# ebanalyse/ebnerd-benchmark

Hardware: AMD Instinct MI355X
Metric: training impressions/sec (higher is better)
Workload: dtype f32

## Files before the change

### ebnerd-benchmark_amd/csrc/ebn_encoder.hip

```cpp
#include "ebn_common.h"

#define EBN_TRY(call)            \
  do {                           \
    int rc__ = (call);           \
    if (rc__ != EBN_OK) return rc__; \
  } while (0)

static int check_dims(const ebn_encoder_dims* d) {
  EBN_REQUIRE(d, EBN_ERR_BAD_ARG);
  EBN_REQUIRE(d->n_seq >= 0 && d->L > 0 && d->Din > 0 && d->h > 0 && d->d > 0 && d->A > 0, EBN_ERR_BAD_ARG);
  return EBN_OK;
}

extern "C" int ebn_encoder_fwd_f32(const ebn_encoder_dims* dims, const ebn_encoder_params* p,
                                   const ebn_encoder_acts* a, const ebn_encoder_scratch* s,
                                   const ebn_step_state* st, ebn_stream_t stream) {
  EBN_TRY(check_dims(dims));
  EBN_REQUIRE(p && a && p->Wqkv && p->W && p->b && p->q, EBN_ERR_BAD_ARG);
  EBN_REQUIRE(a->X && a->QKV && a->Y && a->U && a->w && a->out, EBN_ERR_BAD_ARG);
  const int64_t R = dims->n_seq * dims->L;
  const int E = dims->h * dims->d;
  if (R == 0) return EBN_OK;
  float* ws = s ? s->gemm_ws : nullptr;
  const int64_t ws_n = s ? s->gemm_ws_floats : 0;
  EBN_TRY(ebn_gemm_f32_site(0, 0, R, 3 * E, dims->Din, 1.0f, a->X, dims->Din, p->Wqkv, 3 * E, 0.0f, a->QKV, 3 * E, ws, ws_n,
                            1, stream));
  EBN_TRY(ebn_attn_fwd_f32(a->QKV, 3 * E, a->Y, E, dims->n_seq, dims->L, dims->h, dims->d, st, dims->drop_site,
                           dims->drop_p, stream));
  EBN_TRY(ebn_gemm_f32_ws(0, 0, R, dims->A, E, 1.0f, a->Y, E, p->W, dims->A, 0.0f, a->U, dims->A, ws, ws_n, stream));
  EBN_TRY(ebn_attpool_fwd_f32(a->U, p->b, p->q, a->Y, a->out, a->w, dims->n_seq, dims->L, E, dims->A, stream));
  return EBN_OK;
}

extern "C" int ebn_encoder_fwd_gather_f32(const ebn_encoder_dims* dims, const ebn_encoder_params* p, const ebn_encoder_acts* a,
                                          const ebn_encoder_scratch* s, const int32_t* ids, const float* table, int64_t table_rows,
                                          int32_t* oob_flag, ebn_stream_t stream) {
  EBN_TRY(check_dims(dims));
  EBN_REQUIRE(p && a && ids && table && p->Wqkv && p->W && p->b && p->q, EBN_ERR_BAD_ARG);
  EBN_REQUIRE(a->QKV && a->Y && a->U && a->w && a->out, EBN_ERR_BAD_ARG);
  EBN_REQUIRE(dims->drop_p <= 0.0f, EBN_ERR_UNSUPPORTED);
  const int64_t R = dims->n_seq * dims->L;
  const int E = dims->h * dims->d;
  if (R == 0) return EBN_OK;
  float* ws = s ? s->gemm_ws : nullptr;
  const int64_t ws_n = s ? s->gemm_ws_floats : 0;
  EBN_TRY(ebn_gemm_f32_rowmap(ids, table_rows, R, 3 * E, dims->Din, table, dims->Din, p->Wqkv, 3 * E, a->QKV, 3 * E, oob_flag, stream));
  EBN_TRY(ebn_attn_fwd_f32(a->QKV, 3 * E, a->Y, E, dims->n_seq, dims->L, dims->h, dims->d, nullptr, -1, 0.0f, stream));
  EBN_TRY(ebn_gemm_f32_ws(0, 0, R, dims->A, E, 1.0f, a->Y, E, p->W, dims->A, 0.0f, a->U, dims->A, ws, ws_n, stream));
  EBN_TRY(ebn_attpool_fwd_f32(a->U, p->b, p->q, a->Y, a->out, a->w, dims->n_seq, dims->L, E, dims->A, stream));
  return EBN_OK;
}

extern "C" int ebn_encoder_bwd_f32(const ebn_encoder_dims* dims, const ebn_encoder_params* p,
                                   const ebn_encoder_acts* a, const float* dout, const ebn_encoder_grads* g,
                                   const ebn_encoder_scratch* s, float* dX, int32_t accumulate,
                                   const ebn_step_state* st, ebn_stream_t stream) {
  EBN_TRY(check_dims(dims));
  EBN_REQUIRE(p && a && g && s && dout, EBN_ERR_BAD_ARG);
  EBN_REQUIRE(p->Wqkv && p->W && p->q, EBN_ERR_BAD_ARG);
  EBN_REQUIRE(a->X && a->QKV && a->Y && a->U && a->w, EBN_ERR_BAD_ARG);
  EBN_REQUIRE(g->dWqkv && g->dW && g->db && g->dq, EBN_ERR_BAD_ARG);
  EBN_REQUIRE(s->dY && s->dQKV && s->de && s->partials, EBN_ERR_BAD_ARG);
  const int64_t R = dims->n_seq * dims->L;
  const int E = dims->h * dims->d;
  const int A = dims->A;
  if (R == 0) return EBN_OK;
  const float beta = accumulate ? 1.0f : 0.0f;
  EBN_TRY(ebn_attpool_bwd_pool_f32(a->Y, a->w, dout, nullptr, s->de, dims->n_seq, dims->L, E, stream));
  EBN_TRY(ebn_attpool_bwd_dpre_f32(a->U, p->q, s->de, g->dq, g->db, s->partials, R, A, accumulate, stream));
  const bool fold = ebn_attn_bwd_pooled_supported(dims->L, dims->d) != 0 && (E % 4) == 0 && ebn_aligned16(dout) &&
                    ebn_aligned16(s->dY) && ebn_aligned16(a->QKV) && ebn_aligned16(s->dQKV);
  if (fold) {
    EBN_TRY(ebn_dense_bwd_pair_f32(R, E, A, a->Y, E, a->U, A, p->W, A, beta, g->dW, A, s->dY, E, s->gemm_ws, s->gemm_ws_floats,
                                   stream));
    EBN_TRY(ebn_attn_bwd_pooled_f32(a->QKV, 3 * E, s->dY, E, a->w, dout, E, s->dQKV, 3 * E, dims->n_seq, dims->L, dims->h,
                                    dims->d, st, dims->drop_site, dims->drop_p, stream));
  } else {
    EBN_TRY(ebn_gemm_f32_ws(1, 0, E, A, R, 1.0f, a->Y, E, a->U, A, beta, g->dW, A, s->gemm_ws, s->gemm_ws_floats, stream));
    EBN_TRY(ebn_gemm_f32_rank1(R, E, A, 1.0f, a->U, A, p->W, A, s->dY, E, a->w, dout, E, dims->L, s->gemm_ws,
                               s->gemm_ws_floats, stream));
    EBN_TRY(ebn_attn_bwd_f32(a->QKV, 3 * E, s->dY, E, s->dQKV, 3 * E, dims->n_seq, dims->L, dims->h, dims->d, st, dims->drop_site,
                             dims->drop_p, stream));
  }
  if (dX != nullptr)
    return ebn_dense_bwd_pair_f32(R, dims->Din, 3 * E, a->X, dims->Din, s->dQKV, 3 * E, p->Wqkv, 3 * E, beta, g->dWqkv, 3 * E, dX,
                                  dims->Din, s->gemm_ws, s->gemm_ws_floats, stream);
  EBN_TRY(ebn_gemm_f32_ws(1, 0, dims->Din, 3 * E, R, 1.0f, a->X, dims->Din, s->dQKV, 3 * E, beta, g->dWqkv, 3 * E,
                          s->gemm_ws, s->gemm_ws_floats, stream));
  return EBN_OK;
}

extern "C" int ebn_user_stage_train_f32(const ebn_encoder_dims* dims, const ebn_encoder_params* p, const ebn_encoder_acts* a,
                                        const float* cand, const float* labels, float* scores, float* probs, float* loss_rows,
                                        float* loss_out, float* dcand, float* duser, const ebn_encoder_grads* g,
                                        const ebn_encoder_scratch* s, float* head_partials, float* dX, int32_t C,
                                        int32_t loss_kind, float inv_batch, const ebn_step_state* st, ebn_stream_t stream) {
  EBN_TRY(check_dims(dims));
  EBN_REQUIRE(p && a && g && s && cand && labels && scores && probs && loss_rows && loss_out && dcand && duser && dX, EBN_ERR_BAD_ARG);
  EBN_REQUIRE(p->Wqkv && p->W && p->b && p->q && a->X && a->QKV && a->Y && a->U && a->w && a->out, EBN_ERR_BAD_ARG);
  EBN_REQUIRE(g->dWqkv && g->dW && g->db && g->dq && s->dY && s->dQKV && s->de && s->partials, EBN_ERR_BAD_ARG);
  EBN_REQUIRE(C > 0 && dims->drop_p <= 0.0f, EBN_ERR_BAD_ARG);
  const int64_t B = dims->n_seq, R = dims->n_seq * dims->L;
  const int E = dims->h * dims->d, A = dims->A, L = dims->L;
  if (R == 0) return EBN_OK;
  const bool fused = head_partials != nullptr && ebn_user_head_supported(L, C, E, A) != 0 &&
                     ebn_attn_bwd_pooled_supported(L, dims->d) != 0 && ebn_aligned16(a->U) && ebn_aligned16(a->Y) &&
                     ebn_aligned16(cand) && ebn_aligned16(dcand) && ebn_aligned16(duser) && ebn_aligned16(a->out) &&
                     ebn_aligned16(p->b) && ebn_aligned16(p->q) && ebn_aligned16(s->dY) && ebn_aligned16(a->QKV) &&
                     ebn_aligned16(s->dQKV);
  if (!fused) {
    EBN_TRY(ebn_encoder_fwd_f32(dims, p, a, s, st, stream));
    EBN_TRY(ebn_score_loss_train_f32(cand, a->out, labels, scores, probs, loss_rows, loss_out, dcand, duser, B, C, E, loss_kind,
                                     inv_batch, stream));
    return ebn_encoder_bwd_f32(dims, p, a, duser, g, s, dX, 0, st, stream);
  }
  float* ws = s->gemm_ws;
  const int64_t ws_n = s->gemm_ws_floats;
  EBN_TRY(ebn_gemm_f32_site(0, 0, R, 3 * E, dims->Din, 1.0f, a->X, dims->Din, p->Wqkv, 3 * E, 0.0f, a->QKV, 3 * E, ws, ws_n, 1, stream));
  EBN_TRY(ebn_attn_fwd_f32(a->QKV, 3 * E, a->Y, E, B, L, dims->h, dims->d, nullptr, -1, 0.0f, stream));
  EBN_TRY(ebn_gemm_f32_ws(0, 0, R, A, E, 1.0f, a->Y, E, p->W, A, 0.0f, a->U, A, ws, ws_n, stream));
  EBN_TRY(ebn_user_head_train_f32(a->U, p->b, p->q, a->Y, cand, labels, a->w, a->out, scores, probs, loss_rows, loss_out, dcand,
                                  duser, s->de, g->dq, g->db, head_partials, B, L, C, E, A, loss_kind, inv_batch, stream));
  EBN_TRY(ebn_dense_bwd_pair_f32(R, E, A, a->Y, E, a->U, A, p->W, A, 0.0f, g->dW, A, s->dY, E, ws, ws_n, stream));
  EBN_TRY(ebn_attn_bwd_pooled_f32(a->QKV, 3 * E, s->dY, E, a->w, duser, E, s->dQKV, 3 * E, B, L, dims->h, dims->d, nullptr, -1, 0.0f,
                                  stream));
  return ebn_dense_bwd_pair_f32(R, dims->Din, 3 * E, a->X, dims->Din, s->dQKV, 3 * E, p->Wqkv, 3 * E, 0.0f, g->dWqkv, 3 * E, dX,
                                dims->Din, ws, ws_n, stream);
}
```

### ebnerd-benchmark_amd/csrc/ebn_finish.hip

```cpp
#include "ebn_common.h"
#include "ebn_finish.h"
#include "ebn_reduce.h"

namespace {

struct FinishJobs {
  ebn_finish_job job[EBN_FINISH_MAX_JOBS];
  int32_t first_block[EBN_FINISH_MAX_JOBS + 1];
  int32_t n;
};

struct FinishAdam {
  EbnAdamFlat adam;
  int32_t n_rest;
  int64_t rest_off[EBN_ADAM_FLAT_MAX_REST];
  int64_t rest_len[EBN_ADAM_FLAT_MAX_REST];
  int64_t rest_total;
};
constexpr int REST_PER_BLOCK = 4096;

template <bool ADAM>
__device__ __forceinline__ void grad_finish_body(const FinishJobs& js, const FinishAdam* fa) {
  __shared__ float sm[32][33];
  const EbnAdamFlat* ad = ADAM ? &fa->adam : nullptr;
  if (ADAM && static_cast<int>(blockIdx.x) >= js.first_block[js.n]) {
    const float al = ad->st->adam_alpha;
    const int64_t e0 = static_cast<int64_t>(static_cast<int>(blockIdx.x) - js.first_block[js.n]) * REST_PER_BLOCK;
    for (int64_t e = e0 + threadIdx.x; e < e0 + REST_PER_BLOCK && e < fa->rest_total; e += 1024) {
      int64_t off = e;
      int r = 0;
      while (r + 1 < fa->n_rest && off >= fa->rest_len[r]) off -= fa->rest_len[r++];
      off += fa->rest_off[r];
      ebn_adam_flat_apply(*ad, al, off, ad->grad[off]);
    }
    return;
  }
  int j = 0;
  while (j + 1 < js.n && static_cast<int>(blockIdx.x) >= js.first_block[j + 1]) ++j;
  const ebn_finish_job& q = js.job[j];
  const int blk = static_cast<int>(blockIdx.x) - js.first_block[j], nblk = js.first_block[j + 1] - js.first_block[j];
  if (q.kind == EBN_FINISH_SPLITK) {
    ebn_splitk_sum_body(static_cast<uint32_t>(blk) * 1024u + threadIdx.x, static_cast<uint32_t>(nblk) * 1024u, q.partials, q.n_parts,
                        static_cast<uint32_t>(q.rows * q.cols), static_cast<uint32_t>(q.cols), q.beta, q.out0, q.ld, nullptr, nullptr, 0, 1, nullptr, ad);
  } else if (q.kind == EBN_FINISH_COLRED) {
    ebn_reduce_partials_body(sm, blk, q.partials, q.n_parts, 2, static_cast<int>(q.cols), q.scale, q.out0, q.out1, q.beta != 0.f ? 1 : 0, nullptr,
                             nullptr, ad);
  } else {
    ebn_user_head_finish_body(&sm[0][0], blk, nblk, q.partials, q.rows, static_cast<int>(q.cols), q.out0, q.out1, q.loss_rows, q.loss_out);
    if (ADAM && blk < nblk - 1 && threadIdx.x < 256) {
      const int idx = blk * 256 + static_cast<int>(threadIdx.x), A = static_cast<int>(q.cols);
      if (idx < 2 * A) {
        float* gp = (idx / A == 0 ? q.out0 : q.out1) + (idx % A);
        ebn_adam_flat_apply(*ad, ad->st->adam_alpha, gp - ad->grad, *gp);
      }
    }
  }
}

__global__ __launch_bounds__(1024) void grad_finish_kernel(FinishJobs js) { grad_finish_body<false>(js, nullptr); }
__global__ __launch_bounds__(1024) void grad_finish_adam_kernel(FinishJobs js, FinishAdam fa) { grad_finish_body<true>(js, &fa); }

}

static int plan_jobs(const ebn_finish_job* jobs, int32_t n_jobs, FinishJobs& js) {
  EBN_REQUIRE(n_jobs >= 0 && n_jobs <= EBN_FINISH_MAX_JOBS && (jobs != nullptr || n_jobs == 0), EBN_ERR_BAD_ARG);
  js.n = 0;
  js.first_block[0] = 0;
  for (int32_t i = 0; i < n_jobs; ++i) {
    const ebn_finish_job& q = jobs[i];
    EBN_REQUIRE(q.kind >= EBN_FINISH_SPLITK && q.kind <= EBN_FINISH_HEAD && q.rows >= 0 && q.cols >= 0 && q.n_parts >= 0, EBN_ERR_BAD_ARG);
    if (q.rows == 0 || q.cols == 0) continue;
    EBN_REQUIRE(q.partials && q.out0, EBN_ERR_BAD_ARG);
    int64_t blocks;
    if (q.kind == EBN_FINISH_SPLITK) {
      EBN_REQUIRE(q.n_parts >= 1 && q.ld >= q.cols, EBN_ERR_BAD_ARG);
      EBN_REQUIRE(q.rows * q.cols < (int64_t{1} << 31), EBN_ERR_UNSUPPORTED);
      blocks = ebn_ceil_div(q.rows * q.cols, 1024);
      if (blocks > 16384) blocks = 16384;
    } else if (q.kind == EBN_FINISH_COLRED) {
      EBN_REQUIRE(q.out1 && q.cols < (1 << 24), EBN_ERR_BAD_ARG);
      blocks = ebn_ceil_div(2 * q.cols, 32);
    } else {
      EBN_REQUIRE(q.out1 && q.loss_rows && q.loss_out && q.cols < (1 << 24), EBN_ERR_BAD_ARG);
      blocks = ebn_ceil_div(2 * q.cols, 256) + 1;
    }
    js.job[js.n] = q;
    js.first_block[js.n + 1] = js.first_block[js.n] + static_cast<int32_t>(blocks);
    ++js.n;
  }
  return EBN_OK;
}

extern "C" int ebn_grad_finish_f32(const ebn_finish_job* jobs, int32_t n_jobs, ebn_stream_t stream) {
  FinishJobs js;
  const int rc = plan_jobs(jobs, n_jobs, js);
  if (rc != EBN_OK) return rc;
  if (js.n == 0) return EBN_OK;
  EBN_LAUNCH(grad_finish_kernel, dim3(static_cast<unsigned>(js.first_block[js.n])), dim3(1024), 0, ebn_stream(stream), js);
  EBN_CHECK_LAUNCH();
  return EBN_OK;
}

extern "C" int ebn_grad_finish_adam_f32(const ebn_finish_job* jobs, int32_t n_jobs, const ebn_adam_flat* a, const ebn_step_state* st,
                                        ebn_stream_t stream) {
  EBN_REQUIRE(a != nullptr && st != nullptr && a->theta && a->grad && a->m && a->v && a->numel > 0, EBN_ERR_BAD_ARG);
  EBN_REQUIRE(a->n_rest >= 0 && a->n_rest <= EBN_ADAM_FLAT_MAX_REST, EBN_ERR_BAD_ARG);
  FinishJobs js;
  const int rc = plan_jobs(jobs, n_jobs, js);
  if (rc != EBN_OK) return rc;
  auto inside = [&](const float* p, int64_t count) { return p >= a->grad && count >= 0 && (p - a->grad) + count <= a->numel; };
  for (int i = 0; i < js.n; ++i) {
    const ebn_finish_job& q = js.job[i];
    if (q.kind == EBN_FINISH_SPLITK) EBN_REQUIRE(inside(q.out0, (q.rows - 1) * q.ld + q.cols), EBN_ERR_BAD_ARG);
    else EBN_REQUIRE(inside(q.out0, q.cols) && inside(q.out1, q.cols), EBN_ERR_BAD_ARG);
  }
  FinishAdam fa{};
  fa.adam = EbnAdamFlat{a->grad, a->theta, a->m, a->v, st, static_cast<float>(1.0 - a->beta1), static_cast<float>(1.0 - a->beta2),
                        static_cast<float>(a->eps), a->grad_scale};
  fa.n_rest = a->n_rest;
  for (int i = 0; i < a->n_rest; ++i) {
    EBN_REQUIRE(a->rest_off[i] >= 0 && a->rest_len[i] >= 0 && a->rest_off[i] + a->rest_len[i] <= a->numel, EBN_ERR_BAD_ARG);
    fa.rest_off[i] = a->rest_off[i];
    fa.rest_len[i] = a->rest_len[i];
    fa.rest_total += a->rest_len[i];
  }
  const int64_t blocks = js.first_block[js.n] + ebn_ceil_div(fa.rest_total, REST_PER_BLOCK);
  EBN_REQUIRE(blocks < (int64_t{1} << 30), EBN_ERR_UNSUPPORTED);
  if (blocks == 0) return EBN_OK;
  EBN_LAUNCH(grad_finish_adam_kernel, dim3(static_cast<unsigned>(blocks)), dim3(1024), 0, ebn_stream(stream), js, fa);
  EBN_CHECK_LAUNCH();
  return EBN_OK;
}
```

### ebnerd-benchmark_amd/csrc/ebn_userhead.hip

```cpp
#include "ebn_common.h"
#include "ebn_finish.h"

namespace {

constexpr int HEAD_THREADS = 1024;
constexpr float HEAD_KERAS_EPS = 1e-7f;

struct HeadArgs {
  float* U;
  const float* b;
  const float* q;
  const float* X;
  const float* cand;
  const float* labels;
  float* w;
  float* user;
  float* scores;
  float* probs;
  float* loss_rows;
  float* dcand;
  float* duser;
  float* de;
  float* partials;
  int L, C, E, A, loss_kind;
  float inv_batch;
};

__device__ __forceinline__ float head_bce_probs(float p, float y, float* dldp) {
  const float lo = HEAD_KERAS_EPS, hi = 1.0f - HEAD_KERAS_EPS;
  const bool in_range = p >= lo && p <= hi;
  const float pc = fminf(fmaxf(p, lo), hi);
  const float a = pc + HEAD_KERAS_EPS, bb = 1.0f - pc + HEAD_KERAS_EPS;
  *dldp = in_range ? (-(y / a) + (1.0f - y) / bb) : 0.f;
  return -(y * logf(a) + (1.0f - y) * logf(bb));
}

__global__ __launch_bounds__(HEAD_THREADS) void user_head_train_kernel(HeadArgs a) {
  extern __shared__ __attribute__((aligned(16))) float sm[];
  const int L = a.L, C = a.C, E = a.E, A = a.A;
  float* T = sm;
  float* Xs = T + L * A;
  float* Cs = Xs + L * E;
  float* us = Cs + C * E;
  float* du = us + E;
  float* ev = du + E;
  float* dwv = ev + L;
  float* sc = dwv + L;
  float* dsv = sc + C;
  const int64_t bi = blockIdx.x;
  const int tid = threadIdx.x, lane = tid & 63, wave = tid >> 6;
  const int A4 = A >> 2, E4 = E >> 2;
  {
    const float4* Ug = reinterpret_cast<const float4*>(a.U + bi * L * A);
    const float4* Xg = reinterpret_cast<const float4*>(a.X + bi * L * E);
    const float4* Cg = reinterpret_cast<const float4*>(a.cand + bi * C * E);
    const float4* bg = reinterpret_cast<const float4*>(a.b);
    constexpr int NB = 2;
    for (int base = 0; base < L * E4; base += HEAD_THREADS * NB) {
      float4 v[NB];
#pragma unroll
      for (int j = 0; j < NB; ++j) {
        const int i = base + j * HEAD_THREADS + tid;
        v[j] = Xg[i < L * E4 ? i : L * E4 - 1];
      }
#pragma unroll
      for (int j = 0; j < NB; ++j) {
        const int i = base + j * HEAD_THREADS + tid;
        if (i < L * E4) reinterpret_cast<float4*>(Xs)[i] = v[j];
      }
    }
    for (int base = 0; base < C * E4; base += HEAD_THREADS * NB) {
      float4 v[NB];
#pragma unroll
      for (int j = 0; j < NB; ++j) {
        const int i = base + j * HEAD_THREADS + tid;
        v[j] = Cg[i < C * E4 ? i : C * E4 - 1];
      }
#pragma unroll
      for (int j = 0; j < NB; ++j) {
        const int i = base + j * HEAD_THREADS + tid;
        if (i < C * E4) reinterpret_cast<float4*>(Cs)[i] = v[j];
      }
    }
    for (int base = 0; base < L * A4; base += HEAD_THREADS * NB) {
      float4 v[NB], bb[NB];
#pragma unroll
      for (int j = 0; j < NB; ++j) {
        const int i = base + j * HEAD_THREADS + tid;
        const int ic = i < L * A4 ? i : L * A4 - 1;
        v[j] = Ug[ic];
        bb[j] = bg[ic % A4];
      }
#pragma unroll
      for (int j = 0; j < NB; ++j) {
        const int i = base + j * HEAD_THREADS + tid;
        float4 t;
        t.x = tanhf(v[j].x + bb[j].x);
        t.y = tanhf(v[j].y + bb[j].y);
        t.z = tanhf(v[j].z + bb[j].z);
        t.w = tanhf(v[j].w + bb[j].w);
        if (i < L * A4) reinterpret_cast<float4*>(T)[i] = t;
      }
    }
  }
  __syncthreads();
  for (int l = wave; l < L; l += HEAD_THREADS / 64) {
    float part = 0.f;
    for (int k4 = lane; k4 < A4; k4 += 64) {
      const float4 t = reinterpret_cast<const float4*>(T + l * A)[k4];
      const float4 qq = reinterpret_cast<const float4*>(a.q)[k4];
      part = fmaf(t.w, qq.w, fmaf(t.z, qq.z, fmaf(t.y, qq.y, fmaf(t.x, qq.x, part))));
    }
    part = ebn_wave_sum(part);
    if (lane == 0) ev[l] = part;
  }
  __syncthreads();
  if (wave == 0) {
    float s = 0.f;
    for (int l = lane; l < L; l += 64) {
      const float ex = expf(ev[l]);
      ev[l] = ex;
      s += ex;
    }
    s = ebn_wave_sum(s) + HEAD_KERAS_EPS;
    for (int l = lane; l < L; l += 64) {
      const float wl = ev[l] / s;
      ev[l] = wl;
      a.w[bi * L + l] = wl;
    }
  }
  __syncthreads();
  for (int c4 = tid; c4 < E4; c4 += HEAD_THREADS) {
    float4 acc = make_float4(0.f, 0.f, 0.f, 0.f);
    for (int l = 0; l < L; ++l) {
      const float wl = ev[l];
      const float4 x = reinterpret_cast<const float4*>(Xs + l * E)[c4];
      acc.x = fmaf(wl, x.x, acc.x);
      acc.y = fmaf(wl, x.y, acc.y);
      acc.z = fmaf(wl, x.z, acc.z);
      acc.w = fmaf(wl, x.w, acc.w);
    }
    reinterpret_cast<float4*>(us)[c4] = acc;
    reinterpret_cast<float4*>(a.user + bi * E)[c4] = acc;
  }
  __syncthreads();
  for (int c = wave; c < C; c += HEAD_THREADS / 64) {
    float part = 0.f;
    for (int e4 = lane; e4 < E4; e4 += 64) {
      const float4 x = reinterpret_cast<const float4*>(Cs + c * E)[e4];
      const float4 u = reinterpret_cast<const float4*>(us)[e4];
      part = fmaf(x.w, u.w, fmaf(x.z, u.z, fmaf(x.y, u.y, fmaf(x.x, u.x, part))));
    }
    part = ebn_wave_sum(part);
    if (lane == 0) sc[c] = part;
  }
  __syncthreads();
  if (wave == 0) {
    const float* y = a.labels + bi * C;
    float mx = -INFINITY, ysum = 0.f;
    for (int c = lane; c < C; c += 64) {
      mx = fmaxf(mx, sc[c]);
      ysum += y[c];
    }
    mx = ebn_wave_max(mx);
    ysum = ebn_wave_sum(ysum);
    float se = 0.f;
    for (int c = lane; c < C; c += 64) se += expf(sc[c] - mx);
    se = ebn_wave_sum(se);
    const float lse = mx + logf(se);
    const float invbc = a.inv_batch / static_cast<float>(C);
    float loss = 0.f, dot = 0.f;
    for (int c = lane; c < C; c += 64) {
      const float s = sc[c];
      a.scores[bi * C + c] = s;
      const float p = expf(s - mx) / se;
      a.probs[bi * C + c] = p;
      float ds;
      if (a.loss_kind == 0) {
        const float logp = s - lse;
        loss -= y[c] * logp;
        ds = (expf(logp) * ysum - y[c]) * a.inv_batch;
      } else if (a.loss_kind == 1) {
        loss += fmaxf(s, 0.f) - s * y[c] + log1pf(expf(-fabsf(s)));
        ds = (1.0f / (1.0f + expf(-s)) - y[c]) * invbc;
      } else {
        loss += head_bce_probs(p, y[c], &ds);
        dot = fmaf(p, ds, dot);
      }
      dsv[c] = ds;
    }
    if (a.loss_kind == 2) {
      dot = ebn_wave_sum(dot);
      for (int c = lane; c < C; c += 64) dsv[c] = (expf(sc[c] - mx) / se) * (dsv[c] - dot) * invbc;
    }
    loss = ebn_wave_sum(loss) * (a.loss_kind == 0 ? a.inv_batch : invbc);
    if (lane == 0) a.loss_rows[bi] = loss;
  }
  __syncthreads();
  for (int e4 = tid; e4 < E4; e4 += HEAD_THREADS) {
    const float4 u = reinterpret_cast<const float4*>(us)[e4];
    float4 acc = make_float4(0.f, 0.f, 0.f, 0.f);
    for (int c = 0; c < C; ++c) {
      const float ds = dsv[c];
      const float4 x = reinterpret_cast<const float4*>(Cs + c * E)[e4];
      acc.x = fmaf(ds, x.x, acc.x);
      acc.y = fmaf(ds, x.y, acc.y);
      acc.z = fmaf(ds, x.z, acc.z);
      acc.w = fmaf(ds, x.w, acc.w);
      reinterpret_cast<float4*>(a.dcand + (bi * C + c) * E)[e4] = make_float4(ds * u.x, ds * u.y, ds * u.z, ds * u.w);
    }
    reinterpret_cast<float4*>(du)[e4] = acc;
    reinterpret_cast<float4*>(a.duser + bi * E)[e4] = acc;
  }
  __syncthreads();
  for (int l = wave; l < L; l += HEAD_THREADS / 64) {
    float part = 0.f;
    for (int e4 = lane; e4 < E4; e4 += 64) {
      const float4 x = reinterpret_cast<const float4*>(Xs + l * E)[e4];
      const float4 g = reinterpret_cast<const float4*>(du)[e4];
      part = fmaf(g.w, x.w, fmaf(g.z, x.z, fmaf(g.y, x.y, fmaf(g.x, x.x, part))));
    }
    part = ebn_wave_sum(part);
    if (lane == 0) dwv[l] = part;
  }
  __syncthreads();
  if (wave == 0) {
    float s = 0.f;
    for (int l = lane; l < L; l += 64) s = fmaf(ev[l], dwv[l], s);
    s = ebn_wave_sum(s);
    for (int l = lane; l < L; l += 64) {
      const float d = ev[l] * (dwv[l] - s);
      dwv[l] = d;
      a.de[bi * L + l] = d;
    }
  }
  __syncthreads();
  for (int k = tid; k < A; k += HEAD_THREADS) {
    const float qk = a.q[k];
    float dq = 0.f, db = 0.f;
    for (int l = 0; l < L; ++l) {
      const float t = T[l * A + k], d = dwv[l];
      dq = fmaf(d, t, dq);
      const float dp = d * qk * (1.0f - t * t);
      a.U[(bi * L + l) * A + k] = dp;
      db += dp;
    }
    a.partials[(bi * 2 + 0) * A + k] = dq;
    a.partials[(bi * 2 + 1) * A + k] = db;
  }
}

__global__ __launch_bounds__(256) void user_head_finish_kernel(const float* __restrict__ partials, int64_t B, int A,
                                                               float* __restrict__ dq, float* __restrict__ db,
                                                               const float* __restrict__ loss_rows,
                                                               float* __restrict__ loss_out) {
  __shared__ float sw[4];
  ebn_user_head_finish_body(sw, blockIdx.x, gridDim.x, partials, B, A, dq, db, loss_rows, loss_out);
}

size_t head_lds_bytes(int L, int C, int E, int A) {
  return sizeof(float) * (static_cast<size_t>(L) * A + static_cast<size_t>(L) * E + static_cast<size_t>(C) * E + 2 * static_cast<size_t>(E) +
                          2 * static_cast<size_t>(L) + 2 * static_cast<size_t>(C));
}

}

extern "C" int ebn_user_head_supported(int32_t L, int32_t C, int32_t E, int32_t A) {
  if (L <= 0 || C <= 0 || E <= 0 || A <= 0 || (E % 4) != 0 || (A % 4) != 0) return 0;
  return head_lds_bytes(L, C, E, A) <= 150 * 1024 ? 1 : 0;
}

extern "C" int64_t ebn_user_head_partials_len(int64_t B, int32_t A) { return ebn_dim_ok(B, A) ? B * 2 * static_cast<int64_t>(A) : 0; }

extern "C" int ebn_user_head_train_f32(float* U, const float* b, const float* q, const float* X, const float* cand,
                                       const float* labels, float* w, float* user, float* scores, float* probs,
                                       float* loss_rows, float* loss_out, float* dcand, float* duser, float* de, float* dq,
                                       float* db, float* partials, int64_t B, int32_t L, int32_t C, int32_t E, int32_t A,
                                       int32_t loss_kind, float inv_batch, ebn_stream_t stream) {
  EBN_REQUIRE(U && b && q && X && cand && labels && w && user && scores && probs && loss_rows && loss_out && dcand && duser &&
                  de && partials && ((dq != nullptr) == (db != nullptr)),
              EBN_ERR_BAD_ARG);
  EBN_REQUIRE(B >= 0 && L > 0 && C > 0 && E > 0 && A > 0, EBN_ERR_BAD_ARG);
  EBN_REQUIRE(loss_kind >= 0 && loss_kind <= 2 && ebn_user_head_supported(L, C, E, A), EBN_ERR_UNSUPPORTED);
  EBN_REQUIRE(ebn_aligned16(U) && ebn_aligned16(b) && ebn_aligned16(q) && ebn_aligned16(X) && ebn_aligned16(cand) &&
                  ebn_aligned16(user) && ebn_aligned16(dcand) && ebn_aligned16(duser),
              EBN_ERR_ALIGN);
  if (B == 0) return EBN_OK;
  hipStream_t s = ebn_stream(stream);
  const size_t lds = head_lds_bytes(L, C, E, A);
  static const hipError_t attr = hipFuncSetAttribute(reinterpret_cast<const void*>(&user_head_train_kernel),
                                                     hipFuncAttributeMaxDynamicSharedMemorySize, 150 * 1024);
  if (attr != hipSuccess) return static_cast<int>(attr);
  HeadArgs a{U, b, q, X, cand, labels, w, user, scores, probs, loss_rows, dcand, duser, de, partials, L, C, E, A, loss_kind, inv_batch};
  EBN_LAUNCH(user_head_train_kernel, dim3(static_cast<unsigned>(B)), dim3(HEAD_THREADS), lds, s, a);
  EBN_CHECK_LAUNCH();
  if (dq == nullptr) return EBN_OK;
  EBN_LAUNCH(user_head_finish_kernel, dim3(static_cast<unsigned>(ebn_ceil_div(2 * A, 256) + 1)), dim3(256), 0, s, partials, B, A,
                     dq, db, loss_rows, loss_out);
  EBN_CHECK_LAUNCH();
  return EBN_OK;
}
```

### ebnerd-benchmark_amd/ebrec/models/newsrec/_engine.py

```python
from __future__ import annotations

import ctypes
import math

import numpy as np
import torch

from ebrec import _hip

BETA1, BETA2, ADAM_EPS = 0.9, 0.999, 1e-7
_ALIGN = 64

from ._engine_segments import SegmentsMixin
from ._engine_staging import StagingMixin

LOSS_KIND = {"cross_entropy_loss": 0, "log_loss": 1}
BCE_ON = ("logits", "probs")


def loss_kind_of(loss: str, bce_on: str) -> int:
    if bce_on not in BCE_ON:
        raise ValueError(f"bce_on must be one of {BCE_ON}, got {bce_on}")
    return 0 if loss == "cross_entropy_loss" else (1 if bce_on == "logits" else 2)


def require_gpu() -> torch.device:
    if not torch.cuda.is_available():
        raise RuntimeError("the MI355X NRMS path needs a visible GPU (no CPU fallback); "
                           "torch.cuda.is_available() is False")
    _hip.lib()
    return torch.device("cuda", torch.cuda.current_device())


def eval_loss_from_news(eng, news_all: torch.Tensor, his_idx, pred_idx, y):
    his_idx, pred_idx = np.asarray(his_idx), np.asarray(pred_idx)
    B, C = his_idx.shape[0], pred_idx.shape[1]
    H, E = his_idx.shape[1], eng.E
    idx = torch.from_numpy(np.ascontiguousarray(np.concatenate([his_idx.reshape(-1), pred_idx.reshape(-1)]), dtype=np.int32)).to(eng.device)
    NE = torch.empty(B * (H + C), E, device=eng.device)
    S = _hip.stream_handle
    _hip.call("ebn_gather_rows_f32", _hip.ptr(idx), _hip.ptr(news_all), _hip.ptr(NE), B * (H + C), E, news_all.shape[0], None, -1,
              ctypes.c_float(0.0), None, S())
    user = eng.encode_users_from_news(NE[: B * H].view(B, H, E))
    cand = NE[B * H:]
    scores, probs = torch.empty(B, C, device=eng.device), torch.empty(B, C, device=eng.device)
    _hip.call("ebn_score_fwd_f32", _hip.ptr(cand), _hip.ptr(user), _hip.ptr(scores), _hip.ptr(probs), B, C, E, 0, S())
    labels = (y if isinstance(y, torch.Tensor) else torch.from_numpy(np.ascontiguousarray(np.asarray(y, dtype=np.float32))))
    labels = labels.to(device=eng.device, dtype=torch.float32).reshape(B, C).contiguous()
    rows, junk_c, junk_u = torch.empty(B, device=eng.device), torch.empty(B * C, E, device=eng.device), torch.empty(B, E, device=eng.device)
    loss = torch.empty(1, device=eng.device)
    _hip.call("ebn_score_loss_bwd_f32", _hip.ptr(cand), _hip.ptr(user), _hip.ptr(scores), _hip.ptr(labels), _hip.ptr(rows),
              _hip.ptr(junk_c), _hip.ptr(junk_u), B, C, E, eng.loss_kind, ctypes.c_float(1.0 / B), S())
    _hip.call("ebn_sum_f32", _hip.ptr(rows), B, ctypes.c_float(1.0), _hip.ptr(loss), 0, S())
    return loss, probs


def glorot_uniform_np(shape, seed):
    rng = np.random.default_rng(seed)
    lim = math.sqrt(6.0 / (shape[0] + shape[-1]))
    return rng.uniform(-lim, lim, size=shape).astype(np.float32)


class FlatParams:

    def __init__(self, shapes: dict, device):
        self.shapes = dict(shapes)
        self.offsets = {}
        off = 0
        for name, shp in shapes.items():
            self.offsets[name] = off
            off += -(-int(np.prod(shp)) // _ALIGN) * _ALIGN
        self.numel = off
        self.data = torch.zeros(off, device=device)
        self.grad = torch.zeros(off, device=device)
        self.m = torch.zeros(off, device=device)
        self.v = torch.zeros(off, device=device)

    def view(self, name, buf=None):
        buf = self.data if buf is None else buf
        n = int(np.prod(self.shapes[name]))
        return buf[self.offsets[name]: self.offsets[name] + n].view(*self.shapes[name])

    def g(self, name):
        return self.view(name, self.grad)


class EncoderBuffers:

    def __init__(self, n_seq, L, Din, E, A, device, own_input, need_dx):
        R = n_seq * L
        self.n_seq, self.L, self.Din, self.E, self.A, self.R = n_seq, L, Din, E, A, R
        f = lambda *s: torch.empty(*s, device=device)
        self.X = f(R, Din) if own_input else None
        self.QKV, self.Y, self.U, self.w = f(R, 3 * E), f(R, E), f(R, A), f(R)
        self.out = f(n_seq, E)
        self.dY, self.dQKV, self.de = f(R, E), f(R, 3 * E), f(R)
        self.partials = f(int(_hip.lib().ebn_attpool_partials_len(R, A)))
        wsf = _hip.lib().ebn_gemm_workspace_floats
        ws = max(int(wsf(Din, 3 * E, R)), int(wsf(E, A, R)), int(wsf(R, 3 * E, Din)), int(wsf(R, A, E)), int(wsf(R, E, A)),
                 int(wsf(R, Din, 3 * E)), 1)
        self.ws = f(ws)
        self.fwd_scratch = _hip.EncoderScratch(None, None, None, None, self.ws.data_ptr(), self.ws.numel())
        self.dX = f(R, Din) if need_dx else None


class NRMSEngine(StagingMixin, SegmentsMixin):
    def __init__(self, table: np.ndarray, title_size: int, history_size: int, head_num: int, head_dim: int,
                 attention_hidden_dim: int, dropout: float, learning_rate: float, loss: str, seed=None,
                 train_embedding: bool = True, device=None, process_group=None, shard_table: bool = False,
                 shard_mode: str = "alltoall", deterministic: bool = True, units=None, l2: float = 0.0,
                 shard_partition: str | None = None, shard_capacity_factor: float = 1.25, table_grad_exchange: str = "auto",
                 bce_on: str = "logits", precision: str = "exact"):
        self.device = require_gpu() if device is None else torch.device(device)
        if precision not in ("exact", "split"):
            raise ValueError(f"precision must be 'exact' (fp32 MFMA, the default) or 'split' (bf16x6 split on the bf16 matrix pipe, "
                             f"fp32-accurate, fp32 accumulate), got {precision}")
        self.precision = precision
        if loss not in LOSS_KIND:
            raise ValueError(f"this loss not defined {loss}")
        loss_kind_of(loss, bce_on)
        self.bce_on = bce_on
        self.T, self.H = int(title_size), int(history_size)
        self.h, self.d, self.A = int(head_num), int(head_dim), int(attention_hidden_dim)
        self.E = self.h * self.d
        self.p = float(dropout)
        self.loss = loss
        self.seed = seed
        self.train_embedding = bool(train_embedding)
        if table_grad_exchange not in ("auto", "dense", "sparse"):
            raise ValueError(f"table_grad_exchange must be auto | dense | sparse, got {table_grad_exchange}")
        self.table_grad_exchange = table_grad_exchange
        self._sparse_pin = None
        self.pg = process_group
        table = np.ascontiguousarray(table, dtype=np.float32)
        self.V, self.D = table.shape
        self.exchange = None
        if shard_table:
            from ._dist import ShardedTableExchange

            self.exchange = ShardedTableExchange(self.V, self.D, group=process_group, mode=shard_mode, partition=shard_partition,
                                                 capacity_factor=shard_capacity_factor)
            table = self.exchange.shard_of(table)
        self.table = torch.from_numpy(np.ascontiguousarray(table)).to(self.device)
        D, E, A = self.D, self.E, self.A
        self.units = [int(u) for u in units] if units else []
        if self.units and self.precision == "split":
            raise ValueError("precision='split' covers the news encoder without the optional per-token Dense stack "
                             "(newsencoder_units_per_layer); use precision='exact' with it")
        if self.units and self.units[-1] != E:
            raise ValueError(f"newsencoder_units_per_layer must end with head_num*head_dim = {E} (the news vector is dotted with "
                             f"the {E}-wide user vector, nrms.py:201), got {self.units}")
        shapes = {"n_Wqkv": (D, 3 * E)}
        if self.units:
            from ._mlp import MLPStack

            shapes.update(MLPStack.shapes("n_", E, self.units))
        shapes.update({"n_W": (E, A), "n_b": (A,), "n_q": (A,), "u_Wqkv": (E, 3 * E), "u_W": (E, A), "u_b": (A,), "u_q": (A,)})
        self.params = FlatParams(shapes, self.device)
        self._graphs = {}
        self.mlp = MLPStack(self.params, "n_", E, self.units, self.device, l2, on_realloc=lambda: self._graphs.clear()) if self.units else None
        self._init_weights(seed)
        self.deterministic = bool(deterministic)
        if self.train_embedding:
            self.table_grad = torch.zeros_like(self.table)
            self.table_m = torch.zeros_like(self.table)
            self.table_v = torch.zeros_like(self.table)
            if self.deterministic:
                self.table_acc = torch.zeros(self.table.shape, dtype=torch.int64, device=self.device)
        st = _hip.StepState()
        st.step, st.seed, st.lr, st.adam_alpha = 0, (0 if seed is None else int(seed)) & 0xFFFFFFFF, learning_rate, 0.0
        self.state = torch.frombuffer(bytearray(bytes(st)), dtype=torch.uint8).to(self.device)
        self._lr = float(learning_rate)
        self._bufs = {}
        self.oob_flag = torch.zeros(1, dtype=torch.int32, device=self.device)
        self.keep_table_grad = False
        self.range_flag = torch.zeros(1, dtype=torch.int32, device=self.device)
        self.loss_dev = torch.zeros(1, device=self.device)
        self.use_graph = False
        self.fuse_user_head = True
        self.fuse_eval_gather = True
        self.defer_finish = True
        self.atomic_table_grad = False
        self.graph_collectives = False
        self.overlap_collectives = True
        self.skip_collectives = False
        self._pending = []
        self.defer_flag_checks = False
        self.trace = None
        self.world = 1
        if process_group is not None or (torch.distributed.is_available() and torch.distributed.is_initialized()):
            self.world = torch.distributed.get_world_size(process_group)
        self.guard = None
        if self.world > 1:
            from ._dist import LockStepGuard

            self.guard = LockStepGuard(process_group)
        self.force_collectives = False
        self.adam_in_finish = True
        self._adam_done_in_finish = False

    @property
    def multi(self) -> bool:
        return self.world > 1 or self.force_collectives

    @property
    def loss_kind(self) -> int:
        return loss_kind_of(self.loss, self.bce_on)

    def _init_weights(self, seed):
        D, E, A = self.D, self.E, self.A
        s = (lambda: seed) if seed is not None else (lambda: None)
        pv = self.params.view
        with torch.no_grad():
            for pre, din in (("n", D), ("u", E)):
                w = np.concatenate([glorot_uniform_np((din, E), s()) for _ in range(3)], axis=1)
                pv(f"{pre}_Wqkv").copy_(torch.from_numpy(w))
                pv(f"{pre}_W").copy_(torch.from_numpy(glorot_uniform_np((E, A), s())))
                pv(f"{pre}_b").zero_()
                pv(f"{pre}_q").copy_(torch.from_numpy(glorot_uniform_np((A, 1), s())[:, 0]))
        if self.mlp is not None:
            self.mlp.init_weights((lambda k: None) if seed is None else (lambda k: int(seed) * 1000 + k), glorot_uniform_np)

    def weight_names(self):
        base = ["news.emb", "news.attn.WQ", "news.attn.WK", "news.attn.WV"]
        if self.mlp is not None:
            base += self.mlp.weight_names("news")
        return base + ["news.att.W", "news.att.b", "news.att.q", "user.attn.WQ", "user.attn.WK", "user.attn.WV", "user.att.W",
                       "user.att.b", "user.att.q"]

    def get_weights(self):
        E = self.E
        out = [self._full_table().cpu().numpy()]
        for pre in ("n", "u"):
            w = self.params.view(f"{pre}_Wqkv").cpu().numpy()
            out += [w[:, :E].copy(), w[:, E:2 * E].copy(), w[:, 2 * E:].copy()]
            if pre == "n" and self.mlp is not None:
                out += self.mlp.get_weights()
            out += [self.params.view(f"{pre}_W").cpu().numpy(), self.params.view(f"{pre}_b").cpu().numpy(),
                    self.params.view(f"{pre}_q").cpu().numpy().reshape(-1, 1)]
        return out

    def set_weights(self, weights):
        n_mlp = 6 * len(self.units)
        if len(weights) != 13 + n_mlp:
            raise ValueError(f"expected {13 + n_mlp} weight arrays (emb, 2x[WQ,WK,WV,W,b,q]{' + 6 per Dense/BN layer' if n_mlp else ''}), "
                             f"got {len(weights)}")
        w = [np.asarray(a, dtype=np.float32) for a in weights]
        if n_mlp:
            self.mlp.set_weights([torch.from_numpy(np.ascontiguousarray(a)) for a in w[4:4 + n_mlp]])
            w = w[:4] + w[4 + n_mlp:]
        if w[0].shape != (self.V, self.D):
            raise ValueError(f"embedding shape {w[0].shape} != {(self.V, self.D)}")
        with torch.no_grad():
            t0 = w[0] if self.exchange is None else self.exchange.shard_of(w[0])
            self.table.copy_(torch.from_numpy(np.ascontiguousarray(t0)))
            i = 1
            for pre in ("n", "u"):
                self.params.view(f"{pre}_Wqkv").copy_(torch.from_numpy(np.concatenate(w[i:i + 3], axis=1)))
                self.params.view(f"{pre}_W").copy_(torch.from_numpy(w[i + 3]))
                self.params.view(f"{pre}_b").copy_(torch.from_numpy(w[i + 4].reshape(-1)))
                self.params.view(f"{pre}_q").copy_(torch.from_numpy(w[i + 5].reshape(-1)))
                i += 6

    def _full_table(self) -> torch.Tensor:
        if self.exchange is None or self.exchange.world == 1:
            return self.table
        per = self.exchange.per
        mine = torch.zeros(per, self.D, device=self.device)
        mine[: self.table.shape[0]] = self.table
        parts = [torch.empty_like(mine) for _ in range(self.exchange.world)]
        torch.distributed.all_gather(parts, mine, group=self.pg)
        return self.exchange.unshard(parts)

    def count_params(self):
        return self.V * self.D + sum(int(np.prod(s)) for s in self.params.shapes.values()) + 2 * sum(self.units)

    @property
    def _planned(self) -> bool:
        return self.exchange is not None and self.exchange.mode == "alltoall"

    @property
    def _adam_from_acc(self) -> bool:
        return (self.train_embedding and self.deterministic and self.exchange is None and not self.multi
                and not self.keep_table_grad)

    def _sparse_dp(self, n_tok: int) -> bool:
        if not (self.multi and self.train_embedding and self.exchange is None and self.deterministic and not self.keep_table_grad):
            return False
        if self.table_grad_exchange != "auto":
            return self.table_grad_exchange == "sparse"
        return self.pin_table_grad_exchange(n_tok)

    def pin_table_grad_exchange(self, n_tok_full: int) -> bool:
        if self._sparse_pin is None:
            self._sparse_pin = bool(self.world * int(n_tok_full) < self.V)
        return self._sparse_pin

    @property
    def needs_equal_batches(self) -> bool:
        if self.world <= 1:
            return False
        if self.exchange is not None:
            return True
        if not (self.train_embedding and self.deterministic and not self.keep_table_grad):
            return False
        if self.table_grad_exchange != "auto":
            return self.table_grad_exchange == "sparse"
        return True if self._sparse_pin is None else self._sparse_pin

    @property
    def graph_capable(self) -> bool:
        return self.exchange is None or self._planned

    def allreduce_bytes(self, n_tok: int = 0) -> int:
        n = self.params.numel * 4
        if self.train_embedding and self.exchange is None:
            n += n_tok * (4 + self.D * 4) if self._sparse_dp(n_tok) else self.table_grad.numel() * 4
        return n

    def enable_graphs(self, flag=True):
        self.use_graph = bool(flag)
        if not flag:
            self._graphs = {}
        return self

    @property
    def learning_rate(self):
        return self._lr

    @learning_rate.setter
    def learning_rate(self, lr):
        self._lr = float(lr)
        st = self.read_state()
        st.lr = self._lr
        self.state.copy_(torch.frombuffer(bytearray(bytes(st)), dtype=torch.uint8))

    def read_state(self):
        return _hip.StepState.from_buffer_copy(self.state.cpu().numpy().tobytes())

    def _news_bufs(self, N, train):
        key = ("news", train)
        b = self._bufs.get(key)
        if b is None or b.n_seq < N:
            b = EncoderBuffers(N, self.T, self.D, self.E, self.A, self.device, own_input=True,
                               need_dx=train and self.train_embedding)
            b.ids = torch.empty(N * self.T, dtype=torch.int32, device=self.device)
            if self._planned:
                from ._dist import PlannedBuffers

                ws = int(_hip.lib().ebn_shard_plan_workspace_ints(self.V, self.exchange.world))
                b.xb = PlannedBuffers(self.exchange, N * self.T, self.device, need_grad=train and self.train_embedding, ws_ints=ws)
            self._bufs[key] = b
            if train:
                self._graphs.clear()
        return b

    def _user_bufs(self, B, train, H=None):
        H = self.H if H is None else int(H)
        key = ("user", train) if H == self.H else ("user", train, H)
        b = self._bufs.get(key)
        if b is None or b.n_seq < B:
            b = EncoderBuffers(B, H, self.E, self.E, self.A, self.device, own_input=False, need_dx=False)
            self._bufs[key] = b
            if train and H == self.H:
                self._graphs.clear()
        return b

    def _enc_structs(self, pre, b: EncoderBuffers, n_seq, X, drop_site, drop_p):
        pv = self.params.view
        dims = _hip.EncoderDims(n_seq, b.L, b.Din, self.h, self.d, self.A, drop_site, drop_p)
        params = _hip.EncoderParams(pv(f"{pre}_Wqkv").data_ptr(), pv(f"{pre}_W").data_ptr(),
                                    pv(f"{pre}_b").data_ptr(), pv(f"{pre}_q").data_ptr())
        acts = _hip.EncoderActs(X.data_ptr(), b.QKV.data_ptr(), b.Y.data_ptr(), b.U.data_ptr(), b.w.data_ptr(),
                                b.out.data_ptr())
        return dims, params, acts

    def _encoder_fwd(self, pre, b, n_seq, X, train, n_first=None):
        site, p = (1, self.p) if (train and pre == "n" and self.p > 0) else (-1, 0.0)
        st = _hip.ptr(self.state) if train else None
        if pre == "n" and self.mlp is not None:
            return self._news_encoder_fwd_mlp(b, n_seq, X, train, n_seq if n_first is None else n_first)
        if pre == "n" and self.precision == "split":
            return self._news_encoder_fwd_split(b, n_seq, X, st, site, p)
        dims, params, acts = self._enc_structs(pre, b, n_seq, X, site, p)
        _hip.call("ebn_encoder_fwd_f32", ctypes.byref(dims), ctypes.byref(params), ctypes.byref(acts),
                  ctypes.byref(self._fwd_scratch(b)), st, _hip.stream_handle())

    @staticmethod
    def _fwd_scratch(b):
        return b.fwd_scratch

    def _news_encoder_fwd_mlp(self, b, n_seq, X, train, n_first):
        S, E, A, T = _hip.stream_handle, self.E, self.A, b.L
        R = n_seq * T
        pv = self.params.view
        _hip.call("ebn_gemm_f32_site", 0, 0, R, 3 * E, b.Din, ctypes.c_float(1.0), _hip.ptr(X), b.Din, _hip.ptr(pv("n_Wqkv")), 3 * E,
                  ctypes.c_float(0.0), _hip.ptr(b.QKV), 3 * E, _hip.ptr(b.ws), b.ws.numel(), 1, S())
        _hip.call("ebn_attn_fwd_f32", _hip.ptr(b.QKV), 3 * E, _hip.ptr(b.Y), E, n_seq, T, self.h, self.d, None, -1, ctypes.c_float(0.0), S())
        b.Z = self.mlp.forward(b.Y, n_first * T, (n_seq - n_first) * T, train, self.state, self.p)
        _hip.call("ebn_gemm_f32_ws", 0, 0, R, A, E, ctypes.c_float(1.0), _hip.ptr(b.Z), E, _hip.ptr(pv("n_W")), A, ctypes.c_float(0.0),
                  _hip.ptr(b.U), A, _hip.ptr(b.ws), b.ws.numel(), S())
        _hip.call("ebn_attpool_fwd_f32", _hip.ptr(b.U), _hip.ptr(pv("n_b")), _hip.ptr(pv("n_q")), _hip.ptr(b.Z), _hip.ptr(b.out),
                  _hip.ptr(b.w), n_seq, T, E, A, S())

    def _news_encoder_bwd_mlp(self, b, n_seq, X, dout, dX, n_first):
        S, E, A, T = _hip.stream_handle, self.E, self.A, b.L
        R = n_seq * T
        pv, g = self.params.view, self.params.g
        ws, wsn = _hip.ptr(b.ws), b.ws.numel()
        one, zero = ctypes.c_float(1.0), ctypes.c_float(0.0)
        _hip.call("ebn_attpool_bwd_pool_f32", _hip.ptr(b.Z), _hip.ptr(b.w), _hip.ptr(dout), _hip.ptr(b.dY), _hip.ptr(b.de), n_seq, T, E, S())
        _hip.call("ebn_attpool_bwd_dpre_f32", _hip.ptr(b.U), _hip.ptr(pv("n_q")), _hip.ptr(b.de), _hip.ptr(g("n_q")), _hip.ptr(g("n_b")),
                  _hip.ptr(b.partials), R, A, 0, S())
        _hip.call("ebn_gemm_f32_ws", 1, 0, E, A, R, one, _hip.ptr(b.Z), E, _hip.ptr(b.U), A, zero, _hip.ptr(g("n_W")), A, ws, wsn, S())
        _hip.call("ebn_gemm_f32_ws", 0, 1, R, E, A, one, _hip.ptr(b.U), A, _hip.ptr(pv("n_W")), A, one, _hip.ptr(b.dY), E, ws, wsn, S())
        dYattn = self.mlp.backward(b.dY, b.Y, n_first * T, (n_seq - n_first) * T, self.state, self.p, need_dx0=True,
                                   loss_dev=self.loss_dev)
        _hip.call("ebn_attn_bwd_f32", _hip.ptr(b.QKV), 3 * E, _hip.ptr(dYattn), E, _hip.ptr(b.dQKV), 3 * E, n_seq, T, self.h, self.d,
                  None, -1, ctypes.c_float(0.0), S())
        _hip.call("ebn_gemm_f32_ws", 1, 0, b.Din, 3 * E, R, one, _hip.ptr(X), b.Din, _hip.ptr(b.dQKV), 3 * E, zero, _hip.ptr(g("n_Wqkv")),
                  3 * E, ws, wsn, S())
        if dX is not None:
            _hip.call("ebn_gemm_f32_ws", 0, 1, R, b.Din, 3 * E, one, _hip.ptr(b.dQKV), 3 * E, _hip.ptr(pv("n_Wqkv")), 3 * E, zero,
                      _hip.ptr(dX), b.Din, ws, wsn, S())

    def _split_ws(self, b):
        if getattr(b, "split_ws", None) is None:
            f = _hip.lib().ebn_gemm_prec_workspace_bytes
            R, E3, D = b.R, 3 * b.E, b.Din
            nbytes = max(int(f(R, E3, D, 1)), int(f(D, E3, R, 1)), int(f(R, D, E3, 1)) if b.dX is not None else 0)
            b.split_ws = torch.empty(nbytes // 4 + 64, device=self.device)
            b.split_ws_bytes = nbytes
        return b.split_ws

    def _split_bufs(self, b):
        sb = getattr(b, "split_bufs", None)
        if sb is None:
            L = _hip.lib()
            R, E3, D = b.R, 3 * b.E, b.Din
            u8 = lambda n: torch.empty(int(n) + 64, dtype=torch.uint8, device=self.device)
            sb = b.split_bufs = {"XN": u8(L.ebn_planes_bytes(R, D)), "XT": u8(L.ebn_planes_bytes(D, R)), "Wp": u8(L.ebn_planes_bytes(E3, D)),
                                 "dQp": u8(L.ebn_planes_bytes(E3, R)),
                                 "part": torch.empty(max(int(L.ebn_gemm_planes_workspace_floats(D, E3, R)), int(L.ebn_gemm_planes_workspace_floats(R, E3, D)), 1),
                                                     device=self.device)}
        return sb

    def _gemm_prec(self, b, tA, tB, M, N, K, A, lda, Bm, ldb, C, ldc):
        ws = self._split_ws(b)
        _hip.call("ebn_gemm_f32_prec", tA, tB, M, N, K, ctypes.c_float(1.0), _hip.ptr(A), lda, _hip.ptr(Bm), ldb, ctypes.c_float(0.0),
                  _hip.ptr(C), ldc, _hip.ptr(ws), b.split_ws_bytes, 1, _hip.stream_handle())

    def _news_encoder_fwd_split_gemm(self, b, R):
        S, E = _hip.stream_handle, self.E
        sb = self._split_bufs(b)
        _hip.call("ebn_split_planes_f32", _hip.ptr(self.params.view("n_Wqkv")), 3 * E, 3 * E, b.Din, 1, _hip.ptr(sb["Wp"]), S())
        _hip.call("ebn_gemm_planes_f32", _hip.ptr(sb["XN"]), R, _hip.ptr(sb["Wp"]), 3 * E, b.Din, ctypes.c_float(1.0), ctypes.c_float(0.0),
                  _hip.ptr(b.QKV), 3 * E, _hip.ptr(sb["part"]), sb["part"].numel(), S())

    def _news_encoder_fwd_split(self, b, n_seq, X, st, site, p):
        S, E, A, T = _hip.stream_handle, self.E, self.A, b.L
        R = n_seq * T
        pv = self.params.view
        if getattr(b, "planes_rows", -1) == R:
            self._news_encoder_fwd_split_gemm(b, R)
        else:
            self._gemm_prec(b, 0, 0, R, 3 * E, b.Din, X, b.Din, pv("n_Wqkv"), 3 * E, b.QKV, 3 * E)
        _hip.call("ebn_attn_fwd_f32", _hip.ptr(b.QKV), 3 * E, _hip.ptr(b.Y), E, n_seq, T, self.h, self.d, st, site, ctypes.c_float(p), S())
        _hip.call("ebn_gemm_f32_ws", 0, 0, R, A, E, ctypes.c_float(1.0), _hip.ptr(b.Y), E, _hip.ptr(pv("n_W")), A, ctypes.c_float(0.0),
                  _hip.ptr(b.U), A, _hip.ptr(b.ws), b.ws.numel(), S())
        _hip.call("ebn_attpool_fwd_f32", _hip.ptr(b.U), _hip.ptr(pv("n_b")), _hip.ptr(pv("n_q")), _hip.ptr(b.Y), _hip.ptr(b.out),
                  _hip.ptr(b.w), n_seq, T, E, A, S())

    def _news_encoder_bwd_split(self, b, n_seq, X, dout, dX, site, p):
        self._news_bwd_p1(b, n_seq, dout)
        self._news_bwd_p2(b, n_seq, X, dout, site, p)
        if dX is not None:
            self._news_bwd_p3(b, n_seq, dX)

    def _news_bwd_p1(self, b, n_seq, dout):
        S, E, A, T = _hip.stream_handle, self.E, self.A, b.L
        R = n_seq * T
        pv, g = self.params.view, self.params.g
        ws, wsn = _hip.ptr(b.ws), b.ws.numel()
        one, zero = ctypes.c_float(1.0), ctypes.c_float(0.0)
        _hip.call("ebn_attpool_bwd_pool_f32", _hip.ptr(b.Y), _hip.ptr(b.w), _hip.ptr(dout), None, _hip.ptr(b.de), n_seq, T, E, S())
        _hip.call("ebn_attpool_bwd_dpre_f32", _hip.ptr(b.U), _hip.ptr(pv("n_q")), _hip.ptr(b.de), _hip.ptr(g("n_q")), _hip.ptr(g("n_b")),
                  _hip.ptr(b.partials), R, A, 0, S())
        if self._fold_pooling(T):
            _hip.call("ebn_dense_bwd_pair_f32", R, E, A, _hip.ptr(b.Y), E, _hip.ptr(b.U), A, _hip.ptr(pv("n_W")), A, zero, _hip.ptr(g("n_W")), A,
                      _hip.ptr(b.dY), E, ws, wsn, S())
        else:
            _hip.call("ebn_gemm_f32_ws", 1, 0, E, A, R, one, _hip.ptr(b.Y), E, _hip.ptr(b.U), A, zero, _hip.ptr(g("n_W")), A, ws, wsn, S())
            _hip.call("ebn_gemm_f32_rank1", R, E, A, one, _hip.ptr(b.U), A, _hip.ptr(pv("n_W")), A, _hip.ptr(b.dY), E, _hip.ptr(b.w), _hip.ptr(dout), E,
                      T, ws, wsn, S())

    def _fold_pooling(self, T) -> bool:
        return int(_hip.lib().ebn_attn_bwd_pooled_supported(T, self.d)) != 0 and self.E % 4 == 0

    def _news_bwd_p2(self, b, n_seq, X, dout, site, p):
        S, E, T = _hip.stream_handle, self.E, b.L
        R = n_seq * T
        g = self.params.g
        st = _hip.ptr(self.state)
        one, zero = ctypes.c_float(1.0), ctypes.c_float(0.0)
        if self._fold_pooling(T):
            _hip.call("ebn_attn_bwd_pooled_f32", _hip.ptr(b.QKV), 3 * E, _hip.ptr(b.dY), E, _hip.ptr(b.w), _hip.ptr(dout), E, _hip.ptr(b.dQKV), 3 * E,
                      n_seq, T, self.h, self.d, st, site, ctypes.c_float(p), S())
        else:
            _hip.call("ebn_attn_bwd_f32", _hip.ptr(b.QKV), 3 * E, _hip.ptr(b.dY), E, _hip.ptr(b.dQKV), 3 * E, n_seq, T, self.h, self.d, st, site,
                      ctypes.c_float(p), S())
        if self.precision != "split":
            _hip.call("ebn_gemm_f32_ws", 1, 0, b.Din, 3 * E, R, one, _hip.ptr(X), b.Din, _hip.ptr(b.dQKV), 3 * E, zero, _hip.ptr(g("n_Wqkv")), 3 * E,
                      _hip.ptr(b.ws), b.ws.numel(), S())
        elif getattr(b, "planes_rows", -1) == R:
            sb = self._split_bufs(b)
            _hip.call("ebn_split_planes_f32", _hip.ptr(b.dQKV), 3 * E, 3 * E, R, 1, _hip.ptr(sb["dQp"]), S())
            _hip.call("ebn_gemm_planes_f32", _hip.ptr(sb["XT"]), b.Din, _hip.ptr(sb["dQp"]), 3 * E, R, one, zero, _hip.ptr(g("n_Wqkv")), 3 * E,
                      _hip.ptr(sb["part"]), sb["part"].numel(), S())
        else:
            self._gemm_prec(b, 1, 0, b.Din, 3 * E, R, X, b.Din, b.dQKV, 3 * E, g("n_Wqkv"), 3 * E)

    def _news_bwd_p3(self, b, n_seq, dX):
        E, R = self.E, n_seq * b.L
        pv = self.params.view
        if self.precision != "split":
            _hip.call("ebn_gemm_f32_ws", 0, 1, R, b.Din, 3 * E, ctypes.c_float(1.0), _hip.ptr(b.dQKV), 3 * E, _hip.ptr(pv("n_Wqkv")), 3 * E,
                      ctypes.c_float(0.0), _hip.ptr(dX), b.Din, _hip.ptr(b.ws), b.ws.numel(), _hip.stream_handle())
        else:
            self._gemm_prec(b, 0, 1, R, b.Din, 3 * E, b.dQKV, 3 * E, pv("n_Wqkv"), 3 * E, dX, b.Din)

    def roofline_kernels(self, B, C):
        N = B * (self.H + C)
        nb, _ub = self._train_bufs(B, C)
        S, E, R = _hip.stream_handle, self.E, N * self.T
        pv = self.params.view
        site, p = (0, self.p) if self.p > 0 else (-1, 0.0)
        st = _hip.ptr(self.state)

        def qkv_gemm():
            if self.precision == "split":
                nb.planes_rows = R
                return self._news_encoder_fwd_split_gemm(nb, R)
            _hip.call("ebn_gemm_f32_site", 0, 0, R, 3 * E, nb.Din, ctypes.c_float(1.0), _hip.ptr(nb.X), nb.Din,
                      _hip.ptr(pv("n_Wqkv")), 3 * E, ctypes.c_float(0.0), _hip.ptr(nb.QKV), 3 * E, _hip.ptr(nb.ws), nb.ws.numel(), 1, S())

        def make_gather(ids):
            table_rows = self.table.shape[0]
            src = ids if table_rows == self.V else torch.remainder(ids, table_rows).to(torch.int32)

            def gather():
                self._gather_tokens(nb, src, self.table, table_rows, R, st, site, p, True)

            return gather

        return {"qkv_gemm": qkv_gemm, "gather": make_gather}

    def _encoder_bwd(self, pre, b, n_seq, X, dout, dX, n_first=None):
        if pre == "n" and self.mlp is not None:
            return self._news_encoder_bwd_mlp(b, n_seq, X, dout, dX, n_seq if n_first is None else n_first)
        site, p = (1, self.p) if (pre == "n" and self.p > 0) else (-1, 0.0)
        if pre == "n" and self.precision == "split":
            return self._news_encoder_bwd_split(b, n_seq, X, dout, dX, site, p)
        dims, params, acts = self._enc_structs(pre, b, n_seq, X, site, p)
        g = self.params.g
        grads = _hip.EncoderGrads(g(f"{pre}_Wqkv").data_ptr(), g(f"{pre}_W").data_ptr(), g(f"{pre}_b").data_ptr(),
                                  g(f"{pre}_q").data_ptr())
        scratch = _hip.EncoderScratch(b.dY.data_ptr(), b.dQKV.data_ptr(), b.de.data_ptr(), b.partials.data_ptr(),
                                      b.ws.data_ptr(), b.ws.numel())
        _hip.call("ebn_encoder_bwd_f32", ctypes.byref(dims), ctypes.byref(params), ctypes.byref(acts), _hip.ptr(dout),
                  ctypes.byref(grads), ctypes.byref(scratch), _hip.ptr(dX), 0, _hip.ptr(self.state),
                  _hip.stream_handle())

    def _news_forward(self, b, N, train, n_first=None, looked_up=False):
        site, p = (0, self.p) if (train and self.p > 0) else (-1, 0.0)
        st = _hip.ptr(self.state) if train else None
        n_tok = N * self.T
        if self._planned:
            if not looked_up:
                for _kind, fn in self._lookup_segments(b, N):
                    fn()
            xb = b.xb
            self._gather_tokens(b, xb.inv, xb.rows, self.exchange.world * self.exchange.capacity(n_tok), n_tok, st, site, p, train)
            return self._encoder_fwd("n", b, N, b.X, train, n_first)
        if self.exchange is not None:
            b.plan = self.exchange.plan(b.ids[: n_tok])
            b.rows_uniq = self.exchange.lookup(b.plan, self._local_gather)
            self._gather_tokens(b, b.plan.inv, b.rows_uniq, b.rows_uniq.shape[0], n_tok, st, site, p, train)
            return self._encoder_fwd("n", b, N, b.X, train, n_first)
        if not train and self.fuse_eval_gather and self.mlp is None and self.precision == "exact":
            dims, params, acts = self._enc_structs("n", b, N, b.X, -1, 0.0)
            rc = _hip.lib().ebn_encoder_fwd_gather_f32(ctypes.byref(dims), ctypes.byref(params), ctypes.byref(acts), ctypes.byref(self._fwd_scratch(b)),
                                                       _hip.ptr(b.ids), _hip.ptr(self.table), self.V, _hip.ptr(self.oob_flag), _hip.stream_handle())
            if rc == 0:
                return
            if rc != -2:
                raise _hip.HipError(f"ebn_encoder_fwd_gather_f32 failed with code {rc}")
        self._gather_tokens(b, b.ids, self.table, self.V, n_tok, st, site, p, train)
        self._encoder_fwd("n", b, N, b.X, train, n_first)

    def _gather_tokens(self, b, ids, table, table_rows, n_tok, st, site, p, train):
        if self.precision == "split" and train and self.mlp is None and n_tok <= b.R:
            sb = self._split_bufs(b)
            _hip.call("ebn_gather_split_planes_f32", _hip.ptr(ids), _hip.ptr(table), n_tok, self.D, table_rows, st, site, ctypes.c_float(p),
                      _hip.ptr(self.oob_flag), _hip.ptr(sb["XN"]), _hip.ptr(sb["XT"]), _hip.stream_handle())
            b.planes_rows = n_tok
            return
        b.planes_rows = -1
        _hip.call("ebn_gather_rows_f32", _hip.ptr(ids), _hip.ptr(table), _hip.ptr(b.X), n_tok, self.D, table_rows, st, site,
                  ctypes.c_float(p), _hip.ptr(self.oob_flag), _hip.stream_handle())

    def encode_news(self, ids, chunk=8192) -> torch.Tensor:
        ids = ids if isinstance(ids, torch.Tensor) else np.asarray(ids)
        N = ids.shape[0]
        if ids.ndim != 2 or ids.shape[1] != self.T:
            raise ValueError(f"expected ids of shape (N, {self.T}), got {tuple(ids.shape)}")
        out = torch.empty(N, self.E, device=self.device)
        for s in range(0, N, chunk):
            n = min(chunk, N - s)
            b = self._news_bufs(min(chunk, N), False)
            self._upload_ids(b.ids, ids[s:s + n])
            self._news_forward(b, n, False)
            out[s:s + n].copy_(b.out[:n])
        self._check_oob()
        return out

    def encode_users_from_news(self, NEh: torch.Tensor) -> torch.Tensor:
        B, H = NEh.shape[0], NEh.shape[1]
        X = NEh.reshape(B * H, self.E).contiguous()
        b = self._user_bufs(B, False, H)
        self._encoder_fwd("u", b, B, X, False)
        return b.out[:B].clone()

    def encode_users(self, his) -> torch.Tensor:
        his = his if isinstance(his, torch.Tensor) else np.asarray(his)
        B, H = his.shape[0], his.shape[1]
        NEh = self.encode_news(his.reshape(B * H, self.T))
        return self.encode_users_from_news(NEh.view(B, H, self.E))

    def forward(self, his, pred, mode="softmax"):
        his = his if isinstance(his, torch.Tensor) else np.asarray(his)
        pred = pred if isinstance(pred, torch.Tensor) else np.asarray(pred)
        B, C = his.shape[0], pred.shape[1]
        self._check_shapes(his, pred)
        N = B * (self.H + C)
        nb = self._news_bufs(N, False)
        self._upload_ids(nb.ids, his, pred)
        self._news_forward(nb, N, False, B * self.H)
        ub = self._user_bufs(B, False)
        self._encoder_fwd("u", ub, B, nb.out, False)
        scores = torch.empty(B, C, device=self.device)
        probs = torch.empty(B, C, device=self.device)
        cand = nb.out[B * self.H:]
        _hip.call("ebn_score_fwd_f32", _hip.ptr(cand), _hip.ptr(ub.out), _hip.ptr(scores), _hip.ptr(probs), B, C,
                  self.E, 0 if mode == "softmax" else 1, _hip.stream_handle())
        self._check_oob()
        return probs, scores

    def eval_loss(self, his, pred, y):
        probs, scores = self.forward(his, pred, mode="softmax")
        B, C = scores.shape
        labels = (y if isinstance(y, torch.Tensor) else torch.from_numpy(np.ascontiguousarray(np.asarray(y, dtype=np.float32))))
        labels = labels.to(device=self.device, dtype=torch.float32).reshape(B, C).contiguous()
        nb, ub = self._news_bufs(B * (self.H + C), False), self._user_bufs(B, False)
        rows = torch.empty(B, device=self.device)
        junk_c = torch.empty(B * C, self.E, device=self.device)
        junk_u = torch.empty(B, self.E, device=self.device)
        loss = torch.empty(1, device=self.device)
        _hip.call("ebn_score_loss_bwd_f32", _hip.ptr(nb.out[B * self.H:]), _hip.ptr(ub.out), _hip.ptr(scores),
                  _hip.ptr(labels), _hip.ptr(rows), _hip.ptr(junk_c), _hip.ptr(junk_u), B, C, self.E,
                  self.loss_kind, ctypes.c_float(1.0 / B), _hip.stream_handle())
        _hip.call("ebn_sum_f32", _hip.ptr(rows), B, ctypes.c_float(1.0), _hip.ptr(loss), 0, _hip.stream_handle())
        return loss, probs

    def pair_scores(self, user, news, u_idx, n_idx, sigmoid=True):
        n = u_idx.numel()
        out = torch.empty(n, device=self.device)
        _hip.call("ebn_pair_score_f32", _hip.ptr(user), _hip.ptr(news), _hip.ptr(u_idx), _hip.ptr(n_idx),
                  _hip.ptr(out), n, self.E, 1 if sigmoid else 0, _hip.stream_handle())
        return out

    def _check_shapes(self, his, pred):
        if his.ndim != 3 or his.shape[1] != self.H or his.shape[2] != self.T:
            raise ValueError(f"his_input_title must be (B, {self.H}, {self.T}), got {tuple(his.shape)}")
        if pred.ndim != 3 or pred.shape[0] != his.shape[0] or pred.shape[2] != self.T:
            raise ValueError(f"pred_input_title must be (B, C, {self.T}), got {tuple(pred.shape)}")

    def _check_oob(self, collective=None):
        if collective is None:
            if self.defer_flag_checks:
                return
            collective = self.exchange is not None
        collective = bool(collective) and self.multi
        err = None
        if self._planned:
            for key in sorted((k for k, b in self._bufs.items() if hasattr(b, "xb")), key=repr):
                try:
                    self.exchange.check(self._bufs[key].xb, collective=collective)
                except Exception as e:
                    err = err or e
        flags = torch.cat([self.oob_flag, self.range_flag])
        if collective:
            torch.distributed.all_reduce(flags, op=torch.distributed.ReduceOp.MAX, group=self.pg)
        oob, rng_bad = (int(v) for v in flags.cpu().tolist())
        if oob or rng_bad or err is not None:
            self.oob_flag.zero_()
            self.range_flag.zero_()
        if err is not None:
            raise err
        if oob != 0:
            raise IndexError(f"token id out of range [0, {self.V}) for the embedding table")
        if rng_bad != 0:
            raise FloatingPointError("embedding gradient left the range of the deterministic fixed-point accumulator (|sum| >= 2^22 "
                                     "or NaN): the run has diverged; deterministic=False accumulates in fp32 instead")

    def check_oob(self):
        self._check_oob(collective=True)

    def sync_moving_statistics(self) -> None:
        if self.world > 1 and self.mlp is not None:
            self.mlp.sync_moving_statistics(self.pg)

    def l2_penalty(self) -> float:
        return self.mlp.l2_penalty() if self.mlp is not None else 0.0

    def train_step(self, his, pred, y, return_probs=False, indexed=False):
        his = his if isinstance(his, torch.Tensor) else np.asarray(his)
        pred = pred if isinstance(pred, torch.Tensor) else np.asarray(pred)
        B, C = his.shape[0], pred.shape[1]
        advanced = False
        if indexed:
            if his.ndim != 2 or his.shape[1] != self.H or pred.ndim != 2 or pred.shape[0] != B:
                raise ValueError(f"indexed batches must be (B, {self.H}) and (B, C), got {tuple(his.shape)} {tuple(pred.shape)}")
            nb, ub = self._train_bufs(B, C)
            y, advanced = self._stage_indexed(nb, his, pred, y)
        else:
            self._check_shapes(his, pred)
            nb, ub = self._train_bufs(B, C)
            if self._device_batch(his, pred, y):
                nh = his.numel()
                _hip.call("ebn_copy3_advance", _hip.ptr(his), _hip.ptr(nb.ids), nh * 4, _hip.ptr(pred), _hip.ptr(nb.ids[nh:]),
                          pred.numel() * 4, _hip.ptr(y), _hip.ptr(nb.labels), y.numel() * 4, _hip.ptr(self.state), BETA1, BETA2,
                          _hip.stream_handle())
                y, advanced = None, True
            elif not isinstance(his, torch.Tensor) and not isinstance(pred, torch.Tensor) and not isinstance(y, torch.Tensor):
                for a in (his, pred):
                    if a.size and (a.min() < 0 or a.max() >= self.V):
                        raise IndexError(f"token id out of range [0, {self.V}) for the embedding table")
                self._stage_host([his, pred], nb.ids, y, nb.labels)
                y, advanced = None, True
            else:
                self._upload_ids(nb.ids, his, pred)
        if y is not None:
            labels = (y if isinstance(y, torch.Tensor) else torch.from_numpy(np.ascontiguousarray(np.asarray(y, dtype=np.float32))))
            nb.labels[: B * C].copy_(labels.reshape(-1).to(device=self.device, dtype=torch.float32), non_blocking=True)
        if self.use_graph and self.graph_capable:
            key = self._graph_key(B, C, advanced)
            run = self._graphs.get(key)
            if run is None:
                run = self._capture(B, C, advanced)
            if self.trace is not None:
                self.trace.run(run, self._graph_desc.get(key, []))
            else:
                for fn in run:
                    fn()
        elif self.trace is not None:
            segs = self._segments(B, C, advanced)
            self.trace.run([fn for _kind, fn in segs], [self.SEG_KINDS.get(kind, kind) + (f": {fn.what}" if hasattr(fn, "what") else "") for kind, fn in segs])
        else:
            for _kind, fn in self._segments(B, C, advanced):
                fn()
        if return_probs:
            return self.loss_dev, nb.probs[: B * C].view(B, C), nb.labels[: B * C].view(B, C)
        return self.loss_dev

    def _train_bufs(self, B, C):
        N, E = B * (self.H + C), self.E
        nb = self._news_bufs(N, True)
        ub = self._user_bufs(B, True)
        if not hasattr(nb, "dNE"):
            nb.dNE = torch.empty(nb.n_seq, E, device=self.device)
            nb.scores = torch.empty(nb.n_seq, device=self.device)
            nb.probs = torch.empty(nb.n_seq, device=self.device)
            nb.labels = torch.empty(nb.n_seq, device=self.device)
        if self._deferred(C):
            self._defer_bufs(nb)
        if not hasattr(ub, "duser"):
            ub.duser = torch.empty(ub.n_seq, E, device=self.device)
            ub.loss_rows = torch.empty(ub.n_seq, device=self.device)
            ub.head_partials = torch.empty(max(int(_hip.lib().ebn_user_head_partials_len(ub.n_seq, self.A)), 1), device=self.device)
        return nb, ub

    SEG_KINDS = {"k": "kernels", "c": "collective", "a": "collective started asynchronously", "w": "wait for the started collectives"}

    def _fwd_bwd_kernels(self, B, C, sparse_table_grads=False, part="all"):
        H, E = self.H, self.E
        N = B * (H + C)
        S = _hip.stream_handle
        nb, ub = self._train_bufs(B, C)
        st = _hip.ptr(self.state)
        site1, p1 = (1, self.p) if self.p > 0 else (-1, 0.0)
        deferred = self._deferred(C)
        if part in ("all", "a"):
            self._adam_done_in_finish = False
        if part == "b":
            if deferred:
                return self._news_bwd_deferred(nb, ub, B, N, "p2")
            return self._news_bwd_p2(nb, N, nb.X, nb.dNE, site1, p1)
        if part in ("all", "a"):
            if deferred:
                self._news_forward(nb, N, True, B * H, looked_up=True)
                self._user_stage_deferred(B, C, nb, ub)
            else:
                self._fwd_user_stage_kernels(B, C, nb, ub)
        if part == "a":
            if deferred:
                return self._news_bwd_deferred(nb, ub, B, N, "p1")
            return self._news_bwd_p1(nb, N, nb.dNE)
        if part == "all" and deferred:
            self._news_bwd_deferred(nb, ub, B, N, "p1")
            self._adam_done_in_finish = self._adam_fused(C)
            if self._adam_done_in_finish:
                self._news_bwd_deferred(nb, ub, B, N, "p2a")
                if nb.dX is not None:
                    self._news_bwd_p3(nb, N, nb.dX)
                self._news_bwd_deferred(nb, ub, B, N, "p2b")
            else:
                self._news_bwd_deferred(nb, ub, B, N, "p2")
                if nb.dX is not None:
                    self._news_bwd_p3(nb, N, nb.dX)
        elif part == "all":
            self._encoder_bwd("n", nb, N, nb.X, nb.dNE, nb.dX, B * H)
        elif nb.dX is not None:
            self._news_bwd_p3(nb, N, nb.dX)
        self._table_grad_kernels(nb, N, sparse_table_grads)

    def _deferred(self, C) -> bool:
        L = _hip.lib()
        return bool(self.defer_finish and self.mlp is None and self.precision == "exact" and self.fuse_user_head
                    and self._fold_pooling(self.T) and self._fold_pooling(self.H)
                    and int(L.ebn_user_head_supported(self.H, C, self.E, self.A)) != 0)

    def _adam_fused(self, C) -> bool:
        return bool(self.adam_in_finish and not self.multi and self._deferred(C))

    def _adam_flat_args(self):
        a = getattr(self, "_adam_flat", None)
        if a is None:
            P = self.params
            a = _hip.AdamFlat()
            a.theta, a.grad, a.m, a.v, a.numel = P.data.data_ptr(), P.grad.data_ptr(), P.m.data_ptr(), P.v.data_ptr(), P.numel
            a.beta1, a.beta2, a.eps, a.grad_scale = BETA1, BETA2, ADAM_EPS, 1.0
            rest = sorted((P.offsets[k], int(np.prod(P.shapes[k]))) for k in ("u_Wqkv", "u_W"))
            a.n_rest = len(rest)
            for i, (off, n) in enumerate(rest):
                a.rest_off[i], a.rest_len[i] = off, n
            self._adam_flat = a
        return a

    def _defer_bufs(self, nb):
        if getattr(nb, "ws_dw", None) is None:
            L = _hip.lib()
            nb.ws_dw = torch.empty(max(int(L.ebn_gemm_partials_workspace_floats(self.E, self.A, nb.R)), 1), device=self.device)
            nb.ws_dwqkv = torch.empty(max(int(L.ebn_gemm_partials_workspace_floats(self.D, 3 * self.E, nb.R)), 1), device=self.device)
            nb.finish_jobs = {}
        return nb

    def _user_stage_deferred(self, B, C, nb, ub):
        S, H, E, A = _hip.stream_handle, self.H, self.E, self.A
        R = B * H
        pv, g = self.params.view, self.params.g
        ws, wsn = _hip.ptr(ub.ws), ub.ws.numel()
        one, zero = ctypes.c_float(1.0), ctypes.c_float(0.0)
        X, cand, dcand = nb.out, nb.out[B * H:], nb.dNE[B * H:]
        _hip.call("ebn_gemm_f32_site", 0, 0, R, 3 * E, E, one, _hip.ptr(X), E, _hip.ptr(pv("u_Wqkv")), 3 * E, zero, _hip.ptr(ub.QKV), 3 * E, ws, wsn, 1, S())
        _hip.call("ebn_attn_fwd_f32", _hip.ptr(ub.QKV), 3 * E, _hip.ptr(ub.Y), E, B, H, self.h, self.d, None, -1, zero, S())
        _hip.call("ebn_gemm_f32_ws", 0, 0, R, A, E, one, _hip.ptr(ub.Y), E, _hip.ptr(pv("u_W")), A, zero, _hip.ptr(ub.U), A, ws, wsn, S())
        _hip.call("ebn_user_head_train_f32", _hip.ptr(ub.U), _hip.ptr(pv("u_b")), _hip.ptr(pv("u_q")), _hip.ptr(ub.Y), _hip.ptr(cand), _hip.ptr(nb.labels),
                  _hip.ptr(ub.w), _hip.ptr(ub.out), _hip.ptr(nb.scores), _hip.ptr(nb.probs), _hip.ptr(ub.loss_rows), _hip.ptr(self.loss_dev), _hip.ptr(dcand),
                  _hip.ptr(ub.duser), _hip.ptr(ub.de), None, None, _hip.ptr(ub.head_partials), B, H, C, E, A, self.loss_kind, ctypes.c_float(1.0 / B), S())
        _hip.call("ebn_dense_bwd_pair_f32", R, E, A, _hip.ptr(ub.Y), E, _hip.ptr(ub.U), A, _hip.ptr(pv("u_W")), A, zero, _hip.ptr(g("u_W")), A,
                  _hip.ptr(ub.dY), E, ws, wsn, S())
        _hip.call("ebn_attn_bwd_pooled_f32", _hip.ptr(ub.QKV), 3 * E, _hip.ptr(ub.dY), E, _hip.ptr(ub.w), _hip.ptr(ub.duser), E, _hip.ptr(ub.dQKV), 3 * E,
                  B, H, self.h, self.d, None, -1, zero, S())
        _hip.call("ebn_dense_bwd_pair_f32", R, E, 3 * E, _hip.ptr(X), E, _hip.ptr(ub.dQKV), 3 * E, _hip.ptr(pv("u_Wqkv")), 3 * E, zero, _hip.ptr(g("u_Wqkv")),
                  3 * E, _hip.ptr(nb.dNE), E, ws, wsn, S())

    def _news_bwd_deferred(self, nb, ub, B, N, part):
        S, E, A, T, D = _hip.stream_handle, self.E, self.A, self.T, self.D
        R = N * T
        pv, g = self.params.view, self.params.g
        one, zero = ctypes.c_float(1.0), ctypes.c_float(0.0)
        L = _hip.lib()
        self._defer_bufs(nb)
        if part == "p1":
            _hip.call("ebn_attpool_bwd_pool_f32", _hip.ptr(nb.Y), _hip.ptr(nb.w), _hip.ptr(nb.dNE), None, _hip.ptr(nb.de), N, T, E, S())
            _hip.call("ebn_attpool_bwd_dpre_f32", _hip.ptr(nb.U), _hip.ptr(pv("n_q")), _hip.ptr(nb.de), None, None, _hip.ptr(nb.partials), R, A, 0, S())
            n = ctypes.c_int32(0)
            _hip.call("ebn_gemm_f32_partials", 1, 0, E, A, R, one, _hip.ptr(nb.Y), E, _hip.ptr(nb.U), A, _hip.ptr(nb.ws_dw), nb.ws_dw.numel(), ctypes.byref(n), S())
            nb.finish_jobs["dW"] = int(n.value)
            _hip.call("ebn_gemm_f32_ws", 0, 1, R, E, A, one, _hip.ptr(nb.U), A, _hip.ptr(pv("n_W")), A, zero, _hip.ptr(nb.dY), E, _hip.ptr(nb.ws), nb.ws.numel(), S())
            return
        site, p = (1, self.p) if self.p > 0 else (-1, 0.0)
        if part in ("p2", "p2a"):
            _hip.call("ebn_attn_bwd_pooled_f32", _hip.ptr(nb.QKV), 3 * E, _hip.ptr(nb.dY), E, _hip.ptr(nb.w), _hip.ptr(nb.dNE), E, _hip.ptr(nb.dQKV), 3 * E,
                      N, T, self.h, self.d, _hip.ptr(self.state), site, ctypes.c_float(p), S())
            n = ctypes.c_int32(0)
            _hip.call("ebn_gemm_f32_partials", 1, 0, D, 3 * E, R, one, _hip.ptr(nb.X), D, _hip.ptr(nb.dQKV), 3 * E, _hip.ptr(nb.ws_dwqkv), nb.ws_dwqkv.numel(),
                      ctypes.byref(n), S())
            nb.finish_jobs["dWqkv"] = int(n.value)
            if part == "p2a":
                return
        jobs = (_hip.FinishJob * 4)()
        jobs[0] = _hip.FinishJob(_hip.FINISH_COLRED, int(L.ebn_attpool_partials_len(R, A)) // (2 * A), 1, A, nb.partials.data_ptr(), g("n_q").data_ptr(),
                                 g("n_b").data_ptr(), A, 0.0, 1.0, None, None)
        jobs[1] = _hip.FinishJob(_hip.FINISH_HEAD, 1, B, A, ub.head_partials.data_ptr(), g("u_q").data_ptr(), g("u_b").data_ptr(), A, 0.0, 1.0,
                                 ub.loss_rows.data_ptr(), self.loss_dev.data_ptr())
        jobs[2] = _hip.FinishJob(_hip.FINISH_SPLITK, nb.finish_jobs["dW"], E, A, nb.ws_dw.data_ptr(), g("n_W").data_ptr(), None, A, 0.0, 1.0, None, None)
        jobs[3] = _hip.FinishJob(_hip.FINISH_SPLITK, nb.finish_jobs["dWqkv"], D, 3 * E, nb.ws_dwqkv.data_ptr(), g("n_Wqkv").data_ptr(), None, 3 * E, 0.0, 1.0, None, None)
        if part == "p2b":
            _hip.call("ebn_grad_finish_adam_f32", jobs, 4, ctypes.byref(self._adam_flat_args()), _hip.ptr(self.state), S())
        else:
            _hip.call("ebn_grad_finish_f32", jobs, 4, S())

    def _fwd_user_stage_kernels(self, B, C, nb, ub):
        H, E = self.H, self.E
        N = B * (H + C)
        S = _hip.stream_handle
        st = _hip.ptr(self.state)
        self._news_forward(nb, N, True, B * H, looked_up=True)
        cand, dcand = nb.out[B * H:], nb.dNE[B * H:]
        dims, params, acts = self._enc_structs("u", ub, B, nb.out, -1, 0.0)
        g = self.params.g
        grads = _hip.EncoderGrads(g("u_Wqkv").data_ptr(), g("u_W").data_ptr(), g("u_b").data_ptr(), g("u_q").data_ptr())
        scratch = _hip.EncoderScratch(ub.dY.data_ptr(), ub.dQKV.data_ptr(), ub.de.data_ptr(), ub.partials.data_ptr(),
                                      ub.ws.data_ptr(), ub.ws.numel())
        _hip.call("ebn_user_stage_train_f32", ctypes.byref(dims), ctypes.byref(params), ctypes.byref(acts), _hip.ptr(cand),
                  _hip.ptr(nb.labels), _hip.ptr(nb.scores), _hip.ptr(nb.probs), _hip.ptr(ub.loss_rows), _hip.ptr(self.loss_dev),
                  _hip.ptr(dcand), _hip.ptr(ub.duser), ctypes.byref(grads), ctypes.byref(scratch),
                  _hip.ptr(ub.head_partials) if self.fuse_user_head else None, _hip.ptr(nb.dNE), C, self.loss_kind,
                  ctypes.c_float(1.0 / B), st, S())

    def _accumulate_fixed(self, ids, dX, n_tok, st, site, p):
        _hip.call("ebn_embedding_grad_scatter_fixed_atomic" if self.atomic_table_grad else "ebn_embedding_grad_scatter_fixed", _hip.ptr(ids),
                  _hip.ptr(dX), _hip.ptr(self.table_acc), n_tok, self.D, self.V, st, site, ctypes.c_float(p), _hip.ptr(self.range_flag),
                  _hip.stream_handle())

    def _table_grad_kernels(self, nb, N, sparse_table_grads):
        S = _hip.stream_handle
        st = _hip.ptr(self.state)
        if self.train_embedding and not self._planned and not sparse_table_grads:
            if self.exchange is not None or not self.deterministic:
                self.table_grad.zero_()
            site, p = (0, self.p) if self.p > 0 else (-1, 0.0)
            if self.exchange is not None:
                d_uniq = torch.zeros_like(nb.rows_uniq)
                _hip.call("ebn_embedding_grad_scatter_f32", _hip.ptr(nb.plan.inv), _hip.ptr(nb.dX), _hip.ptr(d_uniq),
                          N * self.T, self.D, d_uniq.shape[0], st, site, ctypes.c_float(p), S())
                self.exchange.scatter_grads(nb.plan, d_uniq, self._local_scatter_add)
            elif self.deterministic:
                self._accumulate_fixed(nb.ids, nb.dX, N * self.T, st, site, p)
                if not self._adam_from_acc:
                    _hip.call("ebn_fixed_to_f32", _hip.ptr(self.table_acc), _hip.ptr(self.table_grad), self.table.numel(),
                              _hip.ptr(self.range_flag), S())
            else:
                _hip.call("ebn_embedding_grad_scatter_f32", _hip.ptr(nb.ids), _hip.ptr(nb.dX), _hip.ptr(self.table_grad),
                          N * self.T, self.D, self.V, st, site, ctypes.c_float(p), S())

    def _optimizer_kernels(self, from_acc=None):
        from_acc = self._adam_from_acc if from_acc is None else from_acc
        S = _hip.stream_handle
        st = _hip.ptr(self.state)
        gs = ctypes.c_float(1.0 / self.world)
        P = self.params
        if not self._adam_done_in_finish:
            _hip.call("ebn_adam_keras_step_f32", _hip.ptr(P.data), _hip.ptr(P.grad), _hip.ptr(P.m), _hip.ptr(P.v), P.numel,
                      st, BETA1, BETA2, ADAM_EPS, gs, S())
        if self.train_embedding and from_acc:
            _hip.call("ebn_adam_keras_step_fixed_f32", _hip.ptr(self.table), _hip.ptr(self.table_acc), _hip.ptr(self.table_m),
                      _hip.ptr(self.table_v), self.table.numel(), st, BETA1, BETA2, ADAM_EPS, gs, _hip.ptr(self.range_flag), S())
        elif self.train_embedding:
            _hip.call("ebn_adam_keras_step_f32", _hip.ptr(self.table), _hip.ptr(self.table_grad), _hip.ptr(self.table_m),
                      _hip.ptr(self.table_v), self.table.numel(), st, BETA1, BETA2, ADAM_EPS, gs, S())
```

### ebnerd-benchmark_amd/ebrec/models/newsrec/_engine_segments.py

```python
from __future__ import annotations

import ctypes

import numpy as np
import torch

from ebrec import _hip

BETA1, BETA2, ADAM_EPS = 0.9, 0.999, 1e-7


def _named(kind, fn, what):
    fn.what = what
    return kind, fn


class SegmentsMixin:
    def _lookup_segments(self, b, N):
        ex, n_tok = self.exchange, N * self.T

        def plan(ids, n, cap, ws, slot_rows, inv, counts):
            _hip.call("ebn_shard_plan_i32", _hip.ptr(ids), n, self.V, ex.world, 1 if ex.cyclic else 0, cap, _hip.ptr(ws),
                      _hip.ptr(slot_rows), _hip.ptr(inv), _hip.ptr(counts), _hip.stream_handle())

        def serve(local_rows, out):
            _hip.call("ebn_gather_rows_f32", _hip.ptr(local_rows), _hip.ptr(self.table), _hip.ptr(out), local_rows.numel(), self.D,
                      self.table.shape[0], None, -1, ctypes.c_float(0.0), None, _hip.stream_handle())

        return ex.lookup_segments(b.ids, n_tok, b.xb, plan, serve)

    def _table_grad_segments(self, b, N):
        ex, n_tok = self.exchange, N * self.T
        site, p = (0, self.p) if self.p > 0 else (-1, 0.0)

        def reduce_local(inv, d_slot):
            d_slot.zero_()
            _hip.call("ebn_embedding_grad_scatter_f32", _hip.ptr(inv), _hip.ptr(b.dX), _hip.ptr(d_slot), n_tok, self.D,
                      d_slot.shape[0], _hip.ptr(self.state), site, ctypes.c_float(p), _hip.stream_handle())

        def accumulate(local_rows, grads):
            self.table_grad.zero_()
            _hip.call("ebn_embedding_grad_scatter_f32", _hip.ptr(local_rows), _hip.ptr(grads), _hip.ptr(self.table_grad),
                      local_rows.numel(), self.D, self.table.shape[0], None, -1, ctypes.c_float(0.0), _hip.stream_handle())

        return ex.grad_segments(n_tok, b.xb, reduce_local, accumulate)

    def _local_gather(self, local_rows: torch.Tensor) -> torch.Tensor:
        m = local_rows.numel()
        out = torch.empty(m, self.D, device=self.device)
        if m:
            _hip.call("ebn_gather_rows_f32", _hip.ptr(local_rows), _hip.ptr(self.table), _hip.ptr(out), m, self.D,
                      self.table.shape[0], None, -1, ctypes.c_float(0.0), _hip.ptr(self.oob_flag), _hip.stream_handle())
        return out

    def _local_scatter_add(self, local_rows: torch.Tensor, grads: torch.Tensor) -> None:
        m = local_rows.numel()
        if m:
            _hip.call("ebn_embedding_grad_scatter_f32", _hip.ptr(local_rows), _hip.ptr(grads), _hip.ptr(self.table_grad),
                      m, self.D, self.table.shape[0], None, -1, ctypes.c_float(0.0), _hip.stream_handle())

    def _state_tensors(self):
        ts = [self.params.data, self.params.grad, self.params.m, self.params.v, self.state, self.loss_dev]
        if self.train_embedding:
            ts += [self.table, self.table_grad, self.table_m, self.table_v] + ([self.table_acc] if self.deterministic else [])
        return ts

    def verify_graph_collectives(self, his, pred, y) -> bool:
        if not (self.use_graph and self.graph_capable and self.multi):
            self.graph_collectives = False
            return False
        if torch.distributed.get_backend(self.pg) != "nccl":
            self.graph_collectives = False
            return False
        torch.cuda.synchronize()
        snap = [t.clone() for t in self._state_tensors()]

        def restore():
            for t, s in zip(self._state_tensors(), snap):
                t.copy_(s)

        def one_step(flag):
            self.graph_collectives = flag
            self._graphs.clear()
            self.train_step(his, pred, y)
            restore()
            self.train_step(his, pred, y)
            torch.cuda.synchronize()
            out = [t.clone() for t in self._state_tensors()]
            restore()
            return out

        ok = True
        try:
            ref = one_step(False)
            got = one_step(True)
            ok = all(torch.equal(a, b) for a, b in zip(ref, got))
        except Exception:
            ok = False
            restore()
        verdict = torch.tensor([1 if ok else 0], dtype=torch.int32, device=self.device)
        torch.distributed.all_reduce(verdict, op=torch.distributed.ReduceOp.MIN, group=self.pg)
        self.graph_collectives = bool(int(verdict.item()))
        self._graphs.clear()
        return self.graph_collectives

    def _graph_key(self, B, C, advanced=False):
        return (B, C, advanced, bool(self.adam_in_finish), bool(self.defer_finish), bool(self.multi))

    def _capture(self, B, C, advanced=False):
        torch.cuda.synchronize()
        key = self._graph_key(B, C, advanced)
        segs, run, pool, i = self._segments(B, C, advanced), [], None, 0
        desc = self.__dict__.setdefault("_graph_desc", {}).setdefault(key, [])
        desc.clear()
        if self.graph_collectives and self.multi:
            g = torch.cuda.CUDAGraph()
            with _hip.capture(g):
                for _kind, fn in segs:
                    fn()
            self._graph_objs = getattr(self, "_graph_objs", []) + [g]
            self._graphs[key] = [g.replay]
            desc.append("ONE hipGraph: " + " | ".join(self.SEG_KINDS[k] for k, _fn in segs))
            return self._graphs[key]
        while i < len(segs):
            if segs[i][0] != "k":
                run.append(segs[i][1])
                desc.append(f"{self.SEG_KINDS[segs[i][0]]}: {getattr(segs[i][1], 'what', 'unnamed')} (segment {i} of the step's {len(segs)})")
                i += 1
                continue
            j = i
            while j < len(segs) and segs[j][0] == "k":
                j += 1
            g = torch.cuda.CUDAGraph()
            with _hip.capture(g, pool=pool):
                for _kind, fn in segs[i:j]:
                    fn()
            pool = pool or g.pool()
            run.append(g.replay)
            desc.append(f"hipGraph replay of kernel segments {i}..{j - 1} of the step's {len(segs)}")
            self._graph_objs = getattr(self, "_graph_objs", []) + [g]
            i = j
        self._graphs[key] = run
        return run

    def _segments(self, B, C, advanced=False):
        N = B * (self.H + C)
        nb, _ub = self._train_bufs(B, C)
        multi = self.multi
        segs = [] if advanced else [("k", lambda: _hip.call("ebn_step_advance", _hip.ptr(self.state), BETA1, BETA2, _hip.stream_handle()))]
        if self._planned:
            segs += self._lookup_segments(nb, N)
        sparse = self._sparse_dp(N * self.T)
        if multi and self.mlp is None and self.overlap_collectives and self.train_embedding:
            segs.append(("k", lambda: (self._fwd_bwd_kernels(B, C, sparse, part="a"), self._fwd_bwd_kernels(B, C, sparse, part="b"))))
            segs.append(_named("a", lambda: self._allreduce_async(self.params.grad), "all-reduce of the flat dense-gradient bucket"))
            segs.append(("k", lambda: self._fwd_bwd_kernels(B, C, sparse, part="c")))
            if self._planned:
                segs += self._table_grad_segments(nb, N)
            if self.exchange is None and not sparse:
                segs.append(_named("c", lambda: self._allreduce_table_grad(), "all-reduce of the dense (V, D) table gradient"))
            if sparse:
                segs += self._sparse_table_grad_segments(nb, N)
            segs.append(("w", self._wait_collectives))
        else:
            segs.append(("k", lambda: self._fwd_bwd_kernels(B, C, sparse)))
            if self._planned and self.train_embedding:
                segs += self._table_grad_segments(nb, N)
            if multi:
                segs.append(_named("c", lambda: self._allreduce_grads(dense_table=not sparse),
                                   "all-reduce of the flat dense-gradient bucket" + (" and of the dense table gradient" if (self.train_embedding and self.exchange is None and not sparse) else "")))
            if sparse:
                segs += self._sparse_table_grad_segments(nb, N)
        segs.append(("k", lambda: self._optimizer_kernels(from_acc=self._adam_from_acc or sparse)))
        return segs

    def _allreduce_async(self, t):
        if self.multi and not self.skip_collectives:
            self._pending.append(torch.distributed.all_reduce(t, group=self.pg, async_op=True))

    def _wait_collectives(self):
        for w in self._pending:
            w.wait()
        self._pending = []

    def _allreduce_table_grad(self):
        if self.multi and not self.skip_collectives:
            torch.distributed.all_reduce(self.table_grad, group=self.pg)

    def _sparse_table_grad_segments(self, nb, N):
        n_tok, W = N * self.T, self.world
        if getattr(nb, "ids_all", None) is None or nb.ids_all.numel() < W * n_tok:
            nb.ids_all = torch.empty(W * nb.n_seq * self.T, dtype=torch.int32, device=self.device)
            nb.dX_all = torch.empty(W * nb.n_seq * self.T, self.D, device=self.device)
        ids_all, dX_all = nb.ids_all[: W * n_tok], nb.dX_all[: W * n_tok]
        site, p = (0, self.p) if self.p > 0 else (-1, 0.0)

        def gather():
            if self.skip_collectives:
                return
            torch.distributed.all_gather_into_tensor(ids_all, nb.ids[:n_tok], group=self.pg)
            torch.distributed.all_gather_into_tensor(dX_all, nb.dX[:n_tok], group=self.pg)

        def accumulate():
            for r in range(W):
                self._accumulate_fixed(ids_all[r * n_tok:], dX_all[r * n_tok:], n_tok, _hip.ptr(self.state), site, p)

        return [_named("c", gather, "all-gather of the per-token (id, gradient row) pairs (sparse table-gradient exchange)"), ("k", accumulate)]

    def _allreduce_grads(self, dense_table=True):
        if self.multi and not self.skip_collectives:
            torch.distributed.all_reduce(self.params.grad, group=self.pg)
            if self.train_embedding and self.exchange is None and dense_table:
                torch.distributed.all_reduce(self.table_grad, group=self.pg)
```

### include/ebnerd_hip.h

```cpp
#ifndef EBNERD_HIP_H
#define EBNERD_HIP_H

#include <stdint.h>

#ifdef __cplusplus
extern "C" {
#endif

#define EBN_ABI_VERSION 1

#define EBN_OK 0
#define EBN_ERR_BAD_ARG (-1)
#define EBN_ERR_UNSUPPORTED (-2)
#define EBN_ERR_ALIGN (-3)

typedef void* ebn_stream_t;

#define EBN_SITE_NEWS_IN 0
#define EBN_SITE_NEWS_ATT 1
#define EBN_SITE_MLP0 8
#define EBN_N_SITES 12

typedef struct ebn_step_state {
  uint32_t step;
  uint32_t seed;
  float adam_alpha;
  float lr;
  uint32_t drop_key[EBN_N_SITES];
} ebn_step_state;

int ebn_abi_version(void);
const char* ebn_error_string(int code);
int64_t ebn_launch_count(void);

int ebn_step_advance(ebn_step_state* st, double beta1, double beta2, ebn_stream_t stream);

int ebn_gather_rows_f32(const int32_t* ids, const float* table, float* out, int64_t n_tok,
                        int32_t D, int64_t V, const ebn_step_state* st, int32_t site,
                        float drop_p, int32_t* oob_flag, ebn_stream_t stream);

int ebn_expand_titles_i32(const int32_t* art_idx, const int32_t* token_matrix, int32_t* ids_out,
                          int64_t n_titles, int32_t T, int64_t n_rows, int32_t* oob_flag,
                          ebn_stream_t stream);

int ebn_embedding_grad_scatter_f32(const int32_t* ids, const float* dX, float* dTable,
                                   int64_t n_tok, int32_t D, int64_t V,
                                   const ebn_step_state* st, int32_t site, float drop_p,
                                   ebn_stream_t stream);

int ebn_embedding_grad_scatter_fixed(const int32_t* ids, const float* dX, int64_t* acc, int64_t n_tok,
                                     int32_t D, int64_t V, const ebn_step_state* st, int32_t site,
                                     float drop_p, int32_t* range_flag, ebn_stream_t stream);
int ebn_embedding_grad_scatter_fixed_atomic(const int32_t* ids, const float* dX, int64_t* acc, int64_t n_tok,
                                            int32_t D, int64_t V, const ebn_step_state* st, int32_t site,
                                            float drop_p, int32_t* range_flag, ebn_stream_t stream);
int ebn_fixed_to_f32(int64_t* acc, float* out, int64_t n, int32_t* range_flag, ebn_stream_t stream);
int ebn_adam_keras_step_fixed_f32(float* theta, int64_t* acc, float* m, float* v, int64_t n, const ebn_step_state* st,
                                  double beta1, double beta2, double eps, float grad_scale, int32_t* range_flag,
                                  ebn_stream_t stream);

int64_t ebn_gemm_split_workspace_bytes(int64_t M, int64_t N, int64_t K);
int ebn_gemm_f32_split(int32_t transA, int32_t transB, int64_t M, int64_t N, int64_t K, float alpha, const float* A,
                       int64_t lda, const float* B, int64_t ldb, float beta, float* C, int64_t ldc, void* workspace,
                       int64_t workspace_bytes, ebn_stream_t stream);
int64_t ebn_planes_bytes(int64_t rows, int64_t K);
int ebn_split_planes_f32(const float* src, int64_t ld, int64_t rows, int64_t K, int32_t trans, void* planes,
                         ebn_stream_t stream);
int ebn_gather_split_planes_f32(const int32_t* ids, const float* table, int64_t n_rows, int32_t D, int64_t V,
                                const ebn_step_state* st, int32_t site, float drop_p, int32_t* oob_flag, void* planes_n,
                                void* planes_t, ebn_stream_t stream);
int64_t ebn_gemm_planes_workspace_floats(int64_t M, int64_t N, int64_t K);
int ebn_gemm_planes_f32(const void* a_planes, int64_t M, const void* b_planes, int64_t N, int64_t K, float alpha, float beta,
                        float* C, int64_t ldc, float* workspace, int64_t workspace_floats, ebn_stream_t stream);
int64_t ebn_gemm_prec_workspace_bytes(int64_t M, int64_t N, int64_t K, int32_t precision);
int ebn_gemm_f32_prec(int32_t transA, int32_t transB, int64_t M, int64_t N, int64_t K, float alpha, const float* A,
                      int64_t lda, const float* B, int64_t ldb, float beta, float* C, int64_t ldc, void* workspace,
                      int64_t workspace_bytes, int32_t precision, ebn_stream_t stream);

int64_t ebn_shard_plan_workspace_ints(int64_t V, int32_t world);
int ebn_shard_plan_i32(const int32_t* ids, int64_t n_tok, int64_t V, int32_t world, int32_t cyclic, int64_t cap,
                       int32_t* workspace, int32_t* slot_rows, int32_t* inv, int32_t* counts, ebn_stream_t stream);

int ebn_gemm_f32(int32_t transA, int32_t transB, int64_t M, int64_t N, int64_t K, float alpha,
                 const float* A, int64_t lda, const float* B, int64_t ldb, float beta, float* C,
                 int64_t ldc, ebn_stream_t stream);
int64_t ebn_gemm_workspace_floats(int64_t M, int64_t N, int64_t K);
int ebn_gemm_plan(int64_t M, int64_t N, int64_t K, int64_t workspace_floats, int32_t* bm, int32_t* bn, int32_t* splits);
int ebn_gemm_f32_ws(int32_t transA, int32_t transB, int64_t M, int64_t N, int64_t K, float alpha,
                    const float* A, int64_t lda, const float* B, int64_t ldb, float beta, float* C,
                    int64_t ldc, float* workspace, int64_t workspace_floats, ebn_stream_t stream);

int64_t ebn_gemm_partials_workspace_floats(int64_t M, int64_t N, int64_t K);
int ebn_gemm_f32_partials(int32_t transA, int32_t transB, int64_t M, int64_t N, int64_t K, float alpha, const float* A,
                          int64_t lda, const float* B, int64_t ldb, float* workspace, int64_t workspace_floats,
                          int32_t* n_parts, ebn_stream_t stream);

#define EBN_FINISH_SPLITK 0
#define EBN_FINISH_COLRED 1
#define EBN_FINISH_HEAD 2
#define EBN_FINISH_MAX_JOBS 6
typedef struct {
  int32_t kind;
  int32_t n_parts;
  int64_t rows, cols;
  const float* partials;
  float* out0;
  float* out1;
  int64_t ld;
  float beta, scale;
  const float* loss_rows;
  float* loss_out;
} ebn_finish_job;
int ebn_grad_finish_f32(const ebn_finish_job* jobs, int32_t n_jobs, ebn_stream_t stream);

#define EBN_ADAM_FLAT_MAX_REST 12
typedef struct ebn_adam_flat {
  float* theta;
  const float* grad;
  float* m;
  float* v;
  int64_t numel;
  double beta1, beta2, eps;
  float grad_scale;
  int32_t n_rest;
  int64_t rest_off[EBN_ADAM_FLAT_MAX_REST];
  int64_t rest_len[EBN_ADAM_FLAT_MAX_REST];
} ebn_adam_flat;
int ebn_grad_finish_adam_f32(const ebn_finish_job* jobs, int32_t n_jobs, const ebn_adam_flat* adam, const ebn_step_state* st,
                             ebn_stream_t stream);

int ebn_gemm_f32_site(int32_t transA, int32_t transB, int64_t M, int64_t N, int64_t K, float alpha,
                      const float* A, int64_t lda, const float* B, int64_t ldb, float beta, float* C,
                      int64_t ldc, float* workspace, int64_t workspace_floats, int32_t site,
                      ebn_stream_t stream);

int ebn_attn_fwd_f32(const float* qkv, int64_t ld_qkv, float* out, int64_t ld_out, int64_t n_seq,
                     int32_t L, int32_t h, int32_t d, const ebn_step_state* st, int32_t site,
                     float drop_p, ebn_stream_t stream);
int ebn_attn_bwd_f32(const float* qkv, int64_t ld_qkv, const float* dout, int64_t ld_dout,
                     float* dqkv, int64_t ld_dqkv, int64_t n_seq, int32_t L, int32_t h, int32_t d,
                     const ebn_step_state* st, int32_t site, float drop_p, ebn_stream_t stream);
int ebn_attn_bwd_pooled_f32(const float* qkv, int64_t ld_qkv, const float* dout, int64_t ld_dout, const float* pool_w,
                            const float* pool_dout, int64_t ld_pool, float* dqkv, int64_t ld_dqkv, int64_t n_seq,
                            int32_t L, int32_t h, int32_t d, const ebn_step_state* st, int32_t site, float drop_p,
                            ebn_stream_t stream);
int ebn_attn_bwd_pooled_supported(int32_t L, int32_t d);

int ebn_gemm_f32_rank1(int64_t M, int64_t N, int64_t K, float alpha, const float* A, int64_t lda, const float* B,
                       int64_t ldb, float* C, int64_t ldc, const float* row_scale, const float* seq_rows,
                       int64_t ld_seq, int32_t L, float* workspace, int64_t workspace_floats, ebn_stream_t stream);

int ebn_dense_bwd_pair_f32(int64_t R, int64_t K_in, int64_t N_out, const float* X, int64_t ldx, const float* dY,
                           int64_t lddy, const float* W, int64_t ldw, float beta_w, float* dW, int64_t lddw, float* dX,
                           int64_t lddx, float* workspace, int64_t workspace_floats, ebn_stream_t stream);

int ebn_dense_relu_fwd_f32(int64_t M, int64_t N, int64_t K, const float* A, int64_t lda, const float* B, int64_t ldb,
                           const float* bias, float* C, int64_t ldc, float* workspace, int64_t workspace_floats,
                           ebn_stream_t stream);

int ebn_attpool_fwd_f32(float* U, const float* b, const float* q, const float* X, float* out,
                        float* w, int64_t n_seq, int32_t L, int32_t E, int32_t A,
                        ebn_stream_t stream);
int ebn_attpool_bwd_pool_f32(const float* X, const float* w, const float* dout, float* dX,
                             float* de, int64_t n_seq, int32_t L, int32_t E,
                             ebn_stream_t stream);
int64_t ebn_attpool_partials_len(int64_t R, int32_t A);
int ebn_attpool_bwd_dpre_f32(float* U, const float* q, const float* de, float* dq, float* db,
                             float* partials, int64_t R, int32_t A, int32_t accumulate,
                             ebn_stream_t stream);
typedef struct ebn_encoder_dims {
  int64_t n_seq;
  int32_t L;
  int32_t Din;
  int32_t h, d;
  int32_t A;
  int32_t drop_site;
  float drop_p;
} ebn_encoder_dims;

typedef struct ebn_encoder_params {
  const float* Wqkv;
  const float* W;
  const float* b;
  const float* q;
} ebn_encoder_params;

typedef struct ebn_encoder_acts {
  const float* X;
  float* QKV;
  float* Y;
  float* U;
  float* w;
  float* out;
} ebn_encoder_acts;

typedef struct ebn_encoder_grads {
  float* dWqkv;
  float* dW;
  float* db;
  float* dq;
} ebn_encoder_grads;

typedef struct ebn_encoder_scratch {
  float* dY;
  float* dQKV;
  float* de;
  float* partials;
  float* gemm_ws;
  int64_t gemm_ws_floats;
} ebn_encoder_scratch;

int ebn_encoder_fwd_f32(const ebn_encoder_dims* dims, const ebn_encoder_params* params,
                        const ebn_encoder_acts* acts, const ebn_encoder_scratch* scratch,
                        const ebn_step_state* st, ebn_stream_t stream);
int ebn_encoder_fwd_gather_f32(const ebn_encoder_dims* dims, const ebn_encoder_params* params, const ebn_encoder_acts* acts,
                               const ebn_encoder_scratch* scratch, const int32_t* ids, const float* table, int64_t table_rows,
                               int32_t* oob_flag, ebn_stream_t stream);
int ebn_gemm_f32_rowmap(const int32_t* ids, int64_t table_rows, int64_t M, int64_t N, int64_t K, const float* table,
                        int64_t ldt, const float* B, int64_t ldb, float* C, int64_t ldc, int32_t* oob_flag, ebn_stream_t stream);

int ebn_encoder_bwd_f32(const ebn_encoder_dims* dims, const ebn_encoder_params* params,
                        const ebn_encoder_acts* acts, const float* dout,
                        const ebn_encoder_grads* grads, const ebn_encoder_scratch* scratch,
                        float* dX, int32_t accumulate, const ebn_step_state* st,
                        ebn_stream_t stream);

int ebn_user_stage_train_f32(const ebn_encoder_dims* dims, const ebn_encoder_params* p, const ebn_encoder_acts* a,
                             const float* cand, const float* labels, float* scores, float* probs, float* loss_rows,
                             float* loss_out, float* dcand, float* duser, const ebn_encoder_grads* g,
                             const ebn_encoder_scratch* s, float* head_partials, float* dX, int32_t C, int32_t loss_kind,
                             float inv_batch, const ebn_step_state* st, ebn_stream_t stream);

int ebn_score_fwd_f32(const float* cand, const float* user, float* scores, float* probs,
                      int64_t B, int32_t C, int32_t E, int32_t mode, ebn_stream_t stream);
int ebn_score_loss_bwd_f32(const float* cand, const float* user, const float* scores,
                           const float* labels, float* loss_rows, float* dcand, float* duser,
                           int64_t B, int32_t C, int32_t E, int32_t loss_kind, float inv_batch,
                           ebn_stream_t stream);
int ebn_score_loss_train_f32(const float* cand, const float* user, const float* labels, float* scores, float* probs,
                             float* loss_rows, float* loss_out, float* dcand, float* duser, int64_t B, int32_t C,
                             int32_t E, int32_t loss_kind, float inv_batch, ebn_stream_t stream);
int ebn_user_head_supported(int32_t L, int32_t C, int32_t E, int32_t A);
int64_t ebn_user_head_partials_len(int64_t B, int32_t A);
int ebn_user_head_train_f32(float* U, const float* b, const float* q, const float* X, const float* cand, const float* labels,
                            float* w, float* user, float* scores, float* probs, float* loss_rows, float* loss_out,
                            float* dcand, float* duser, float* de, float* dq, float* db, float* partials, int64_t B,
                            int32_t L, int32_t C, int32_t E, int32_t A, int32_t loss_kind, float inv_batch,
                            ebn_stream_t stream);
int ebn_auc_hist_f32(const float* probs, const float* labels, int64_t n, const double* thresholds, int32_t n_thresholds,
                     int64_t* pos_hist, int64_t* neg_hist, ebn_stream_t stream);
int ebn_pair_score_f32(const float* user, const float* news, const int32_t* u_idx,
                       const int32_t* n_idx, float* out, int64_t n_pairs, int32_t E, int32_t mode,
                       ebn_stream_t stream);

int ebn_adam_keras_step_f32(float* theta, const float* g, float* m, float* v, int64_t n,
                            const ebn_step_state* st, double beta1, double beta2, double eps,
                            float grad_scale, ebn_stream_t stream);

int ebn_bias_relu_f32(const float* X, const float* bias, float* Y, int64_t R, int32_t Ccols,
                      ebn_stream_t stream);
int64_t ebn_colsum_partials_len(int64_t R, int32_t Ccols);
int ebn_bias_relu_bwd_f32(const float* Y, const float* dY, float* dX, float* dbias,
                          float* partials, int64_t R, int32_t Ccols, int32_t accumulate,
                          ebn_stream_t stream);
int ebn_batchnorm_fwd_f32(const float* X, const float* gamma, const float* beta,
                          float* moving_mean, float* moving_var, float* Y, float* xhat,
                          float* mean_out, float* istd_out, float* partials, int64_t R,
                          int32_t Ccols, int32_t training, const ebn_step_state* st,
                          int32_t site, float drop_p, int64_t elem_offset,
                          ebn_stream_t stream);
int ebn_batchnorm_bwd_f32(const float* dY, const float* xhat, const float* gamma,
                          const float* istd, float* dX, float* dgamma, float* dbeta,
                          float* partials, int64_t R, int32_t Ccols, int32_t training,
                          int32_t accumulate, const ebn_step_state* st, int32_t site,
                          float drop_p, int64_t elem_offset, ebn_stream_t stream);
int ebn_batchnorm2_fwd_f32(const float* X, const float* gamma, const float* beta, float* moving_mean, float* moving_var,
                           float* Y, float* xhat, float* mean_out0, float* istd_out0, float* mean_out1, float* istd_out1,
                           int64_t R0, int64_t R1, int32_t Ccols, const ebn_step_state* st, int32_t site, float drop_p,
                           ebn_stream_t stream);
int ebn_batchnorm2_relu_bwd_f32(const float* dY, const float* xhat, const float* relu_out, const float* gamma,
                                const float* istd0, const float* istd1, float* dX, float* dgamma, float* dbeta,
                                float* dbias, int64_t R0, int64_t R1, int32_t Ccols, const ebn_step_state* st, int32_t site,
                                float drop_p, ebn_stream_t stream);

#define EBN_DVN_MAX_LAYERS 4
typedef struct ebn_dvn_args {
  int32_t n_layers, din, e_out;
  int32_t units[EBN_DVN_MAX_LAYERS];
  int32_t n0, n1;
  float drop_p, l2;
  const float* W[EBN_DVN_MAX_LAYERS + 1];
  const float* b[EBN_DVN_MAX_LAYERS + 1];
  const float* gamma[EBN_DVN_MAX_LAYERS];
  const float* beta[EBN_DVN_MAX_LAYERS];
  float* moving_mean[EBN_DVN_MAX_LAYERS];
  float* moving_var[EBN_DVN_MAX_LAYERS];
  const float* X0;
  float* R[EBN_DVN_MAX_LAYERS];
  float* Xn[EBN_DVN_MAX_LAYERS];
  float* NE;
  float* stat;
  const float* dNE;
  float* dY[EBN_DVN_MAX_LAYERS];
  float* dP[EBN_DVN_MAX_LAYERS + 1];
  float* ggamma[EBN_DVN_MAX_LAYERS];
  float* gbeta[EBN_DVN_MAX_LAYERS];
  float* loss;
  int32_t* range_flag;
} ebn_dvn_args;
int ebn_dvn_supported(const ebn_dvn_args* args);
int64_t ebn_dvn_stat_floats(const ebn_dvn_args* args);
int ebn_dvn_fwd_train_f32(const ebn_dvn_args* args, const ebn_step_state* st, ebn_stream_t stream);
int ebn_dvn_bwd_f32(const ebn_dvn_args* args, const ebn_step_state* st, ebn_stream_t stream);

int ebn_docvec_stage_gather_f32(const int32_t* idx0, int64_t n0, const int32_t* idx1, int64_t n1, const float* labels_src,
                                float* labels_dst, int64_t n_labels, const float* matrix, int64_t n_rows, int32_t din, float* X0,
                                int32_t* oob_flag, ebn_step_state* st, double beta1, double beta2, ebn_stream_t stream);

#define EBN_TN_GROUP_MAX 8
typedef struct ebn_tn_problem {
  int64_t M, N, K;
  const float* A;
  int64_t lda;
  const float* B;
  int64_t ldb;
  float* C;
  int64_t ldc;
  float* colsum;
  const float* l2_W;
  float two_lambda;
} ebn_tn_problem;
int ebn_gemm_tn_group_f32(const ebn_tn_problem* problems, int32_t n, ebn_stream_t stream);

#define EBN_DVN_FINALE_MAX_REST 12
typedef struct ebn_dvn_finale {
  float* theta;
  const float* grad;
  float* m;
  float* v;
  int64_t numel;
  double beta1, beta2, eps;
  float grad_scale;
  int32_t n_rest;
  int64_t rest_off[EBN_DVN_FINALE_MAX_REST];
  int64_t rest_len[EBN_DVN_FINALE_MAX_REST];
  const float* head_partials;
  int64_t B;
  int32_t A;
  float* dq;
  float* db;
  const float* loss_rows;
  float* loss_out;
} ebn_dvn_finale;
int ebn_dvn_finale_f32(const ebn_dvn_args* args, const ebn_tn_problem* problems, int32_t n, const ebn_dvn_finale* fin,
                       const ebn_step_state* st, ebn_stream_t stream);

#define EBN_SITE_NPA_CONV 2
#define EBN_SITE_NPA_NEWS_PAP 3
#define EBN_SITE_NPA_USER_PAP 4

int ebn_conv1d_fwd_f32(const float* X, const float* W, const float* bias, float* Vd, int64_t n_titles, int32_t T, int32_t E,
                       int32_t F, int32_t window, const ebn_step_state* st, int32_t conv_site, float conv_p, int32_t pap_site,
                       float pap_p, ebn_stream_t stream);
int ebn_conv1d_bwd_data_f32(const float* dVd, const float* Vd, const float* W, float* dX, int64_t n_titles, int32_t T, int32_t E,
                            int32_t F, int32_t window, const ebn_step_state* st, float conv_p, float pap_p, ebn_stream_t stream);
int ebn_conv1d_wgrad_splits(int64_t n_titles, int32_t T, int32_t E, int32_t F, int32_t window);
int64_t ebn_conv1d_wgrad_workspace_floats(int64_t n_titles, int32_t T, int32_t E, int32_t F, int32_t window, int32_t splits);
int ebn_conv1d_bwd_weight_f32(const float* X, const float* dVd, const float* Vd, float* partials, int32_t splits, int64_t n_titles,
                              int32_t T, int32_t E, int32_t F, int32_t window, const ebn_step_state* st, float conv_p, float pap_p,
                              ebn_stream_t stream);

int ebn_pap_fwd_f32(float* U, const float* ba, const float* Q, const int32_t* q_idx, int64_t n_q, const float* V, float* out,
                    float* w, float* out_d, int64_t n_drop, int64_t n_seq, int32_t L, int32_t F, int32_t A,
                    const ebn_step_state* st, int32_t site, float drop_p, ebn_stream_t stream);
int ebn_pap_bwd_f32(float* U, const float* Q, const int32_t* q_idx, int64_t n_q, const float* V, const float* w, float* dout,
                    float* dV, float* dq, int64_t n_drop, int64_t n_seq, int32_t L, int32_t F, int32_t A,
                    const ebn_step_state* st, int32_t site, float drop_p, ebn_stream_t stream);
int ebn_pap_dq_reduce_f32(const float* dq, const int32_t* q_idx, int64_t n_seq, float* dQ, int64_t n_q, int32_t A,
                          ebn_stream_t stream);

int ebn_attpool_masked_fwd_f32(float* U, const float* b, const float* q, const float* X, const int32_t* ids, float* out,
                               float* w, int64_t n_seq, int32_t L, int32_t E, int32_t A, ebn_stream_t stream);
int ebn_gru_fwd_f32(const float* gx, const float* X, const float* Wrec, const float* bias, const float* h0, float* Hs,
                    float* act, int64_t B, int32_t H, int32_t F, int32_t U, ebn_stream_t stream);
int ebn_gru_bwd_f32(const float* dhH, const float* X, const float* Wrec, const float* Hs, const float* act, float* dgx,
                    float* dgh, float* dh0, int64_t B, int32_t H, int32_t F, int32_t U, ebn_stream_t stream);

#define EBN_SITE_NAML_BODY_IN 5
#define EBN_SITE_NAML_BODY_CONV 6

int ebn_naml_catview_fwd_f32(const int32_t* ids0, const float* table0, int64_t rows0, int32_t K0, const float* Wb0,
                             float* out0, const int32_t* ids1, const float* table1, int64_t rows1, int32_t K1,
                             const float* Wb1, float* out1, int64_t N, int32_t F, int32_t* oob_flag, ebn_stream_t stream);
int64_t ebn_naml_catview_partials_len(int64_t N, int32_t K0, int32_t K1, int32_t F);
int ebn_naml_catview_bwd_f32(const int32_t* ids0, const float* table0, int64_t rows0, int32_t K0, const float* Wb0,
                             const float* out0, const float* dout0, float* dWb0, float* dtable0, const int32_t* ids1,
                             const float* table1, int64_t rows1, int32_t K1, const float* Wb1, const float* out1,
                             const float* dout1, float* dWb1, float* dtable1, float* partials, int64_t partials_len,
                             int64_t N, int32_t F, ebn_stream_t stream);
int ebn_naml_viewatt_fwd_f32(float* U, const float* b, const float* q, const float* Vw, float* w, float* news, int64_t N,
                             int32_t n_views, int32_t F, int32_t A, ebn_stream_t stream);
int ebn_naml_viewatt_bwd_f32(const float* Vw, const float* w, const float* dnews, float* dVw, float* de, int64_t N,
                             int32_t n_views, int32_t F, ebn_stream_t stream);

int ebn_ff_ln_fwd_f32(const float* X, const float* bias, const float* res, const float* gamma, const float* beta, float eps,
                      int32_t mode, uint32_t drop_key, float drop_p, float* Y, float* xhat, float* rstd, int64_t R, int32_t D,
                      ebn_stream_t stream);
int64_t ebn_ff_ln_partials_len(int64_t R, int32_t D);
int ebn_ff_ln_bwd_f32(const float* dY, const float* xhat, const float* rstd, const float* gamma, int32_t mode, uint32_t drop_key,
                      float drop_p, float* dX, float* dres, float* partials, int32_t* n_parts, int64_t R, int32_t D,
                      ebn_stream_t stream);
int ebn_ff_colsum_finish_f32(const float* partials, int64_t n_parts, int64_t stride, int64_t width, float* out,
                             ebn_stream_t stream);
int ebn_ff_gelu_fwd_f32(const float* X, const float* bias, float* Y, int64_t R, int32_t C, ebn_stream_t stream);
int ebn_ff_gelu_bwd_f32(const float* X, const float* bias, const float* dY, float* dX, float* dbias, float* partials, int64_t R,
                        int32_t C, ebn_stream_t stream);
int ebn_ff_pool_fwd_f32(float* U, const float* b1, const float* w2, const float* b2, const float* X, const float* mask, float* out,
                        float* w, float* sinv, int64_t n_seq, int32_t L, int32_t D, ebn_stream_t stream);
int ebn_ff_pool_bwd_f32(const float* X, const float* w, const float* sinv, const float* dout, float* dX, float* de, float* db2n,
                        int64_t n_seq, int32_t L, int32_t D, ebn_stream_t stream);
int ebn_ff_head_fwd_f32(const float* user, const float* cand, const float* W, const float* b, float* score, int64_t N, int32_t D,
                        ebn_stream_t stream);
int ebn_ff_head_bwd_f32(const float* user, const float* cand, const float* W, const float* score, const float* dscore, float* duser,
                        float* dcand, float* dW, float* db, int64_t N, int32_t D, ebn_stream_t stream);
int ebn_ff_attn_fwd_f32(float* Q, float* K, const float* bq, const float* bk, const float* btr, const float* Wqa, const float* bqa,
                        const float* Wka, const float* bka, const float* mask, float* AO, float* SV0, float* qw, float* kw,
                        float* pq, float* pk, int64_t n_seq, int32_t T, int32_t D, int32_t heads, ebn_stream_t stream);
int64_t ebn_ff_attn_partials_len(int64_t n_seq, int32_t D, int32_t heads);
int ebn_ff_attn_supported(int32_t T, int32_t D, int32_t heads, int32_t with_backward);
int ebn_ff_attn_bwd_f32(const float* Q, const float* K, const float* Wqa, const float* Wka, const float* qw, const float* kw,
                        const float* pq, const float* pk, const float* dAO, const float* dSV, float* dQ, float* dK, float* partials,
                        int32_t* n_parts, int64_t n_seq, int32_t T, int32_t D, int32_t heads, ebn_stream_t stream);

int ebn_copy3(const void* s0, void* d0, int64_t n0, const void* s1, void* d1, int64_t n1, const void* s2, void* d2,
              int64_t n2, ebn_stream_t stream);
int ebn_copy3_advance(const void* s0, void* d0, int64_t n0, const void* s1, void* d1, int64_t n1, const void* s2,
                      void* d2, int64_t n2, ebn_step_state* st, double beta1, double beta2, ebn_stream_t stream);

int ebn_axpy_f32(float a, const float* x, float* y, int64_t n, ebn_stream_t stream);
int ebn_l2_reg_f32(const float* W, float* gW, int64_t n, float lambda, float* partials, float* loss,
                   ebn_stream_t stream);
int ebn_l2_reg4_f32(const float* W0, float* g0, int64_t n0, const float* W1, float* g1, int64_t n1, const float* W2,
                    float* g2, int64_t n2, const float* W3, float* g3, int64_t n3, float lambda, float* partials,
                    float* loss, ebn_stream_t stream);
int ebn_sum_f32(const float* x, int64_t n, float scale, float* out, int32_t accumulate,
                ebn_stream_t stream);
int ebn_sumsq_f32(const float* x, int64_t n, float scale, float* out, int32_t accumulate,
                  ebn_stream_t stream);

int ebn_ba_unit_rows_f32(const float* src, float* dst, int64_t n_rows, int64_t D, ebn_stream_t stream);
int ebn_ba_intralist_f32(const float* unit, int64_t n_rows, int64_t D, const int32_t* ids, int64_t n_ids, const int64_t* offsets,
                         int64_t n_lists, int32_t form, float* out, ebn_stream_t stream);
int ebn_ba_cross_f32(const float* unit, int64_t n_rows, int64_t D, const int32_t* ids_r, int64_t n_ids_r, const int64_t* off_r,
                     const int32_t* ids_h, int64_t n_ids_h, const int64_t* off_h, int64_t n_lists, int32_t form, float* out,
                     ebn_stream_t stream);
int ebn_ba_pairdist_f32(const float* unit, int64_t n_rows, int64_t D, const int32_t* ids, int64_t m, float* out, ebn_stream_t stream);
int ebn_ba_list_mean_f32(const float* values, int64_t n_rows, const int32_t* ids, int64_t n_ids, const int64_t* offsets,
                         int64_t n_lists, int32_t transform, float* out, ebn_stream_t stream);
int ebn_ba_subset_sums_f32(const float* dist, int64_t m, const int32_t* subsets, int64_t k, int64_t n_subsets, float* out,
                           ebn_stream_t stream);

#ifdef __cplusplus
}
#endif
#endif
```

Baseline: 25740.

## Fuse user-head dense projection and its backward GEMMs into the head kernel

Adds a dense variant of the user-head training kernel. It computes tanh(XW+b) with MFMA inside the block, and also computes dY = dpre·Wᵀ and per-sequence dW partials in-kernel using an atomic work queue over 16x16 tiles. The dW partials are then reduced by a split-k sum folded into the grad finish job. This removes the separate U GEMM and the dense backward pair GEMMs along with their global round-trips of U. In exchange it needs a B×E×A partial workspace, and the reduction adds traffic proportional to the batch size.

```diff
diff --git a/ebnerd-benchmark_amd/csrc/ebn_encoder.hip b/ebnerd-benchmark_amd/csrc/ebn_encoder.hip
--- a/ebnerd-benchmark_amd/csrc/ebn_encoder.hip
+++ b/ebnerd-benchmark_amd/csrc/ebn_encoder.hip
@@ -127,3 +127,38 @@
   return ebn_dense_bwd_pair_f32(R, dims->Din, 3 * E, a->X, dims->Din, s->dQKV, 3 * E, p->Wqkv, 3 * E, 0.0f, g->dWqkv, 3 * E, dX,
                                 dims->Din, ws, ws_n, stream);
 }
+
+extern "C" int ebn_user_stage_dense_train_f32(const ebn_encoder_dims* dims, const ebn_encoder_params* p, const ebn_encoder_acts* a,
+                                              const float* cand, const float* labels, float* scores, float* probs, float* loss_rows,
+                                              float* loss_out, float* dcand, float* duser, const ebn_encoder_grads* g,
+                                              const ebn_encoder_scratch* s, float* head_partials, float* dW_parts, float* dX,
+                                              int32_t C, int32_t loss_kind, float inv_batch, const ebn_step_state* st,
+                                              ebn_stream_t stream) {
+  EBN_TRY(check_dims(dims));
+  EBN_REQUIRE(p && a && g && s && cand && labels && scores && probs && loss_rows && loss_out && dcand && duser && dX, EBN_ERR_BAD_ARG);
+  EBN_REQUIRE(p->Wqkv && p->W && p->b && p->q && a->X && a->QKV && a->Y && a->U && a->w && a->out, EBN_ERR_BAD_ARG);
+  EBN_REQUIRE(g->dWqkv && g->dW && g->db && g->dq && s->dY && s->dQKV && s->de && s->partials, EBN_ERR_BAD_ARG);
+  EBN_REQUIRE(C > 0 && dims->drop_p <= 0.0f, EBN_ERR_BAD_ARG);
+  const int64_t B = dims->n_seq, R = dims->n_seq * dims->L;
+  const int E = dims->h * dims->d, A = dims->A, L = dims->L;
+  if (R == 0) return EBN_OK;
+  const bool dense = head_partials != nullptr && dW_parts != nullptr &&
+                     ebn_user_head_dense_supported(B, L, C, E, A, p->W, a->Y, s->dY, dW_parts) != 0 &&
+                     ebn_attn_bwd_pooled_supported(L, dims->d) != 0 && ebn_aligned16(cand) && ebn_aligned16(dcand) &&
+                     ebn_aligned16(duser) && ebn_aligned16(a->out) && ebn_aligned16(p->b) && ebn_aligned16(p->q) &&
+                     ebn_aligned16(a->QKV) && ebn_aligned16(s->dQKV);
+  if (!dense)
+    return ebn_user_stage_train_f32(dims, p, a, cand, labels, scores, probs, loss_rows, loss_out, dcand, duser, g, s, head_partials, dX, C,
+                                    loss_kind, inv_batch, st, stream);
+  float* ws = s->gemm_ws;
+  const int64_t ws_n = s->gemm_ws_floats;
+  EBN_TRY(ebn_gemm_f32_site(0, 0, R, 3 * E, dims->Din, 1.0f, a->X, dims->Din, p->Wqkv, 3 * E, 0.0f, a->QKV, 3 * E, ws, ws_n, 1, stream));
+  EBN_TRY(ebn_attn_fwd_f32(a->QKV, 3 * E, a->Y, E, B, L, dims->h, dims->d, nullptr, -1, 0.0f, stream));
+  EBN_TRY(ebn_user_head_dense_train_f32(p->W, p->b, p->q, a->Y, cand, labels, a->w, a->out, scores, probs, loss_rows, loss_out, dcand, duser,
+                                        s->de, g->dq, g->db, head_partials, s->dY, dW_parts, B, L, C, E, A, loss_kind, inv_batch, stream));
+  EBN_TRY(ebn_splitk_sum_f32(dW_parts, static_cast<int32_t>(B), E, A, 0.0f, g->dW, A, stream));
+  EBN_TRY(ebn_attn_bwd_pooled_f32(a->QKV, 3 * E, s->dY, E, a->w, duser, E, s->dQKV, 3 * E, B, L, dims->h, dims->d, nullptr, -1, 0.0f,
+                                  stream));
+  return ebn_dense_bwd_pair_f32(R, dims->Din, 3 * E, a->X, dims->Din, s->dQKV, 3 * E, p->Wqkv, 3 * E, 0.0f, g->dWqkv, 3 * E, dX,
+                                dims->Din, ws, ws_n, stream);
+}
diff --git a/ebnerd-benchmark_amd/csrc/ebn_finish.hip b/ebnerd-benchmark_amd/csrc/ebn_finish.hip
--- a/ebnerd-benchmark_amd/csrc/ebn_finish.hip
+++ b/ebnerd-benchmark_amd/csrc/ebn_finish.hip
@@ -57,6 +57,11 @@
   }
 }
 
+__global__ __launch_bounds__(1024) void splitk_sum_kernel(const float* __restrict__ part, int splits, uint32_t total, uint32_t n32, float beta,
+                                                          float* __restrict__ C, int64_t ldc) {
+  ebn_splitk_sum_body(blockIdx.x * 1024u + threadIdx.x, gridDim.x * 1024u, part, splits, total, n32, beta, C, ldc, nullptr, nullptr, 0, 1, nullptr);
+}
+
 __global__ __launch_bounds__(1024) void grad_finish_kernel(FinishJobs js) { grad_finish_body<false>(js, nullptr); }
 __global__ __launch_bounds__(1024) void grad_finish_adam_kernel(FinishJobs js, FinishAdam fa) { grad_finish_body<true>(js, &fa); }
 
@@ -88,6 +93,20 @@
     js.first_block[js.n + 1] = js.first_block[js.n] + static_cast<int32_t>(blocks);
     ++js.n;
   }
+  return EBN_OK;
+}
+
+extern "C" int ebn_splitk_sum_f32(const float* partials, int32_t n_parts, int64_t rows, int64_t cols, float beta, float* out, int64_t ld,
+                                  ebn_stream_t stream) {
+  EBN_REQUIRE(rows >= 0 && cols >= 0 && n_parts >= 1 && ld >= cols, EBN_ERR_BAD_ARG);
+  if (rows == 0 || cols == 0) return EBN_OK;
+  EBN_REQUIRE(partials && out, EBN_ERR_BAD_ARG);
+  EBN_REQUIRE(rows <= EBN_DIM_MAX && cols <= EBN_DIM_MAX && rows * cols < (int64_t{1} << 31), EBN_ERR_UNSUPPORTED);
+  int64_t blocks = ebn_ceil_div(rows * cols, 1024);
+  if (blocks > 16384) blocks = 16384;
+  EBN_LAUNCH(splitk_sum_kernel, dim3(static_cast<unsigned>(blocks)), dim3(1024), 0, ebn_stream(stream), partials, n_parts,
+             static_cast<uint32_t>(rows * cols), static_cast<uint32_t>(cols), beta, out, ld);
+  EBN_CHECK_LAUNCH();
   return EBN_OK;
 }
 
diff --git a/ebnerd-benchmark_amd/csrc/ebn_userhead.hip b/ebnerd-benchmark_amd/csrc/ebn_userhead.hip
--- a/ebnerd-benchmark_amd/csrc/ebn_userhead.hip
+++ b/ebnerd-benchmark_amd/csrc/ebn_userhead.hip
@@ -1,5 +1,10 @@
 #include "ebn_common.h"
 #include "ebn_finish.h"
+
+typedef float head_f32x4 __attribute__((ext_vector_type(4)));
+typedef int head_i32x4 __attribute__((ext_vector_type(4)));
+__device__ head_f32x4 head_buffer_load_x4(head_i32x4 rsrc, int voffset, int soffset, int aux) __asm("llvm.amdgcn.raw.buffer.load.v4f32");
+__device__ float head_buffer_load_x1(head_i32x4 rsrc, int voffset, int soffset, int aux) __asm("llvm.amdgcn.raw.buffer.load.f32");
 
 namespace {
 
@@ -24,6 +29,9 @@
   float* partials;
   int L, C, E, A, loss_kind;
   float inv_batch;
+  const float* W;
+  float* dY;
+  float* dWparts;
 };
 
 __device__ __forceinline__ float head_bce_probs(float p, float y, float* dldp) {
@@ -35,18 +43,112 @@
   return -(y * logf(a) + (1.0f - y) * logf(bb));
 }
 
-__global__ __launch_bounds__(HEAD_THREADS) void user_head_train_kernel(HeadArgs a) {
+
+
+__device__ __forceinline__ head_i32x4 head_rsrc(const float* base) {
+  const unsigned long long a = reinterpret_cast<unsigned long long>(base);
+  head_i32x4 r;
+  r.x = static_cast<int>(static_cast<uint32_t>(a));
+  r.y = static_cast<int>(static_cast<uint32_t>(a >> 32) & 0xFFFFu);
+  r.z = -1;
+  r.w = 0x00020000;
+  return r;
+}
+
+template <bool B_KC>
+__device__ __forceinline__ void head_b_load(head_f32x4 (&b)[2], head_i32x4 rsrc, int voff, int ldb4, int k0, int kq, int K) {
+  const bool whole = k0 + 32 <= K;
+#pragma unroll
+  for (int h = 0; h < 2; ++h) {
+    const int kg = k0 + 16 * h;
+    if (B_KC) {
+      const int v = (whole || kg + 4 * kq < K) ? voff + kg * 4 : 0;
+      b[h] = head_buffer_load_x4(rsrc, whole ? voff : v, whole ? kg * 4 : 0, 0);
+    } else {
+      const int v = (whole || kg + 4 * kq < K) ? voff + kg * ldb4 : 0;
+#pragma unroll
+      for (int s = 0; s < 4; ++s) b[h][s] = head_buffer_load_x1(rsrc, whole ? voff : v, (whole ? kg * ldb4 : 0) + s * ldb4, 0);
+    }
+  }
+}
+
+__device__ __forceinline__ void head_chunk_mma(head_f32x4& acc0, head_f32x4& acc1, const float* a_row, const head_f32x4 (&b)[2], int k0, int kq, int K) {
+  head_f32x4 a[2], bb[2];
+  if (k0 + 32 <= K) {
+#pragma unroll
+    for (int h = 0; h < 2; ++h) {
+      a[h] = *reinterpret_cast<const head_f32x4*>(a_row + k0 + 16 * h + 4 * kq);
+      bb[h] = b[h];
+    }
+  } else {
+    const head_f32x4 zero = {0.f, 0.f, 0.f, 0.f};
+#pragma unroll
+    for (int h = 0; h < 2; ++h) {
+      const int kk = k0 + 16 * h + 4 * kq;
+      const bool ok = kk < K;
+      const head_f32x4 t = *reinterpret_cast<const head_f32x4*>(a_row + (ok ? kk : 0));
+      a[h] = ok ? t : zero;
+      bb[h] = ok ? b[h] : zero;
+    }
+  }
+#pragma unroll
+  for (int s = 0; s < 4; ++s) {
+    acc0 = __builtin_amdgcn_mfma_f32_16x16x4f32(a[0][s], bb[0][s], acc0, 0, 0, 0);
+    acc1 = __builtin_amdgcn_mfma_f32_16x16x4f32(a[1][s], bb[1][s], acc1, 0, 0, 0);
+  }
+}
+
+template <bool B_KC>
+__device__ __forceinline__ head_f32x4 head_block_mma(const float* a_row, const float* __restrict__ Bg, int ldb, int col, int K, int kq) {
+  head_f32x4 acc0 = {0.f, 0.f, 0.f, 0.f}, acc1 = {0.f, 0.f, 0.f, 0.f};
+  const head_i32x4 rsrc = head_rsrc(Bg);
+  const int ldb4 = ldb * 4;
+  const int voff = B_KC ? (col * ldb + 4 * kq) * 4 : (4 * kq * ldb + col) * 4;
+  head_f32x4 b0[2], b1[2], b2[2];
+  head_b_load<B_KC>(b0, rsrc, voff, ldb4, 0, kq, K);
+  head_b_load<B_KC>(b1, rsrc, voff, ldb4, 32, kq, K);
+  head_b_load<B_KC>(b2, rsrc, voff, ldb4, 64, kq, K);
+  __builtin_amdgcn_sched_barrier(0);
+  for (int k0 = 0; k0 < K; k0 += 96) {
+    head_chunk_mma(acc0, acc1, a_row, b0, k0, kq, K);
+    __builtin_amdgcn_sched_barrier(0);
+    head_b_load<B_KC>(b0, rsrc, voff, ldb4, k0 + 96, kq, K);
+    __builtin_amdgcn_sched_barrier(0);
+    if (k0 + 32 < K) head_chunk_mma(acc0, acc1, a_row, b1, k0 + 32, kq, K);
+    __builtin_amdgcn_sched_barrier(0);
+    head_b_load<B_KC>(b1, rsrc, voff, ldb4, k0 + 128, kq, K);
+    __builtin_amdgcn_sched_barrier(0);
+    if (k0 + 64 < K) head_chunk_mma(acc0, acc1, a_row, b2, k0 + 64, kq, K);
+    __builtin_amdgcn_sched_barrier(0);
+    head_b_load<B_KC>(b2, rsrc, voff, ldb4, k0 + 160, kq, K);
+    __builtin_amdgcn_sched_barrier(0);
+  }
+  return acc0 + acc1;
+}
+
+__host__ __device__ __forceinline__ int head_row_stride(int n) { return ((n >> 2) & 1) ? n : n + 4; }
+
+__device__ __forceinline__ int head_next_task(int* counter, int lane) {
+  int t = 0;
+  if (lane == 0) t = atomicAdd(counter, 1);
+  return __builtin_amdgcn_readfirstlane(t);
+}
+
+template <bool DENSE>
+__device__ __forceinline__ void user_head_body(const HeadArgs& a) {
   extern __shared__ __attribute__((aligned(16))) float sm[];
   const int L = a.L, C = a.C, E = a.E, A = a.A;
   float* T = sm;
-  float* Xs = T + L * A;
-  float* Cs = Xs + L * E;
+  const int XS = DENSE ? head_row_stride(E) : E, TS = DENSE ? head_row_stride(A) : A;
+  float* Xs = T + L * TS;
+  float* Cs = Xs + L * XS;
   float* us = Cs + C * E;
   float* du = us + E;
   float* ev = du + E;
   float* dwv = ev + L;
   float* sc = dwv + L;
   float* dsv = sc + C;
+  int* tasks = reinterpret_cast<int*>(dsv + C);
   const int64_t bi = blockIdx.x;
   const int tid = threadIdx.x, lane = tid & 63, wave = tid >> 6;
   const int A4 = A >> 2, E4 = E >> 2;
@@ -66,7 +168,10 @@
 #pragma unroll
       for (int j = 0; j < NB; ++j) {
         const int i = base + j * HEAD_THREADS + tid;
-        if (i < L * E4) reinterpret_cast<float4*>(Xs)[i] = v[j];
+        if (i < L * E4) {
+          if (DENSE) reinterpret_cast<float4*>(Xs + (i / E4) * XS)[i % E4] = v[j];
+          else reinterpret_cast<float4*>(Xs)[i] = v[j];
+        }
       }
     }
     for (int base = 0; base < C * E4; base += HEAD_THREADS * NB) {
@@ -82,7 +187,7 @@
         if (i < C * E4) reinterpret_cast<float4*>(Cs)[i] = v[j];
       }
     }
-    for (int base = 0; base < L * A4; base += HEAD_THREADS * NB) {
+    for (int base = 0; !DENSE && base < L * A4; base += HEAD_THREADS * NB) {
       float4 v[NB], bb[NB];
 #pragma unroll
       for (int j = 0; j < NB; ++j) {
@@ -102,12 +207,29 @@
         if (i < L * A4) reinterpret_cast<float4*>(T)[i] = t;
       }
     }
-  }
-  __syncthreads();
+    if (DENSE && tid < 2) tasks[tid] = 0;
+  }
+  __syncthreads();
+  if constexpr (DENSE) {
+    const int ln = lane & 15, kq = lane >> 4;
+    const int nrb = (L + 15) >> 4, ncb = (A + 15) >> 4;
+    for (int t = head_next_task(&tasks[0], lane); t < nrb * ncb; t = head_next_task(&tasks[0], lane)) {
+      const int rb = t % nrb, cb = t / nrb;
+      const int arow = min(16 * rb + ln, L - 1), col = 16 * cb + ln, colc = min(col, A - 1);
+      const head_f32x4 acc = head_block_mma<false>(Xs + arow * XS, a.W, A, colc, E, kq);
+      const float bcol = a.b[colc];
+#pragma unroll
+      for (int i = 0; i < 4; ++i) {
+        const int row = 16 * rb + 4 * kq + i;
+        if (row < L && col < A) T[row * TS + col] = tanhf(acc[i] + bcol);
+      }
+    }
+    __syncthreads();
+  }
   for (int l = wave; l < L; l += HEAD_THREADS / 64) {
     float part = 0.f;
     for (int k4 = lane; k4 < A4; k4 += 64) {
-      const float4 t = reinterpret_cast<const float4*>(T + l * A)[k4];
+      const float4 t = reinterpret_cast<const float4*>(T + l * TS)[k4];
       const float4 qq = reinterpret_cast<const float4*>(a.q)[k4];
       part = fmaf(t.w, qq.w, fmaf(t.z, qq.z, fmaf(t.y, qq.y, fmaf(t.x, qq.x, part))));
     }
@@ -134,7 +256,7 @@
     float4 acc = make_float4(0.f, 0.f, 0.f, 0.f);
     for (int l = 0; l < L; ++l) {
       const float wl = ev[l];
-      const float4 x = reinterpret_cast<const float4*>(Xs + l * E)[c4];
+      const float4 x = reinterpret_cast<const float4*>(Xs + l * XS)[c4];
       acc.x = fmaf(wl, x.x, acc.x);
       acc.y = fmaf(wl, x.y, acc.y);
       acc.z = fmaf(wl, x.z, acc.z);
@@ -216,7 +338,7 @@
   for (int l = wave; l < L; l += HEAD_THREADS / 64) {
     float part = 0.f;
     for (int e4 = lane; e4 < E4; e4 += 64) {
-      const float4 x = reinterpret_cast<const float4*>(Xs + l * E)[e4];
+      const float4 x = reinterpret_cast<const float4*>(Xs + l * XS)[e4];
       const float4 g = reinterpret_cast<const float4*>(du)[e4];
       part = fmaf(g.w, x.w, fmaf(g.z, x.z, fmaf(g.y, x.y, fmaf(g.x, x.x, part))));
     }
@@ -239,16 +361,70 @@
     const float qk = a.q[k];
     float dq = 0.f, db = 0.f;
     for (int l = 0; l < L; ++l) {
-      const float t = T[l * A + k], d = dwv[l];
+      const float t = T[l * TS + k], d = dwv[l];
       dq = fmaf(d, t, dq);
       const float dp = d * qk * (1.0f - t * t);
-      a.U[(bi * L + l) * A + k] = dp;
+      if (DENSE) T[l * TS + k] = dp;
+      else a.U[(bi * L + l) * A + k] = dp;
       db += dp;
     }
     a.partials[(bi * 2 + 0) * A + k] = dq;
     a.partials[(bi * 2 + 1) * A + k] = db;
   }
-}
+  if constexpr (DENSE) {
+    __syncthreads();
+    const int ln = lane & 15, kq = lane >> 4;
+    const int nrb = (L + 15) >> 4, neb = (E + 15) >> 4, ncb = (A + 15) >> 4, nch = (ncb + 3) >> 2;
+    const int n_dy = nrb * neb, n_all = n_dy + neb * nch;
+    float* dYg = a.dY + bi * L * E;
+    float* dWg = a.dWparts + bi * E * A;
+    for (int t = head_next_task(&tasks[1], lane); t < n_all; t = head_next_task(&tasks[1], lane)) {
+      if (t < n_dy) {
+        const int rb = t % nrb, eb = t / nrb;
+        const int arow = min(16 * rb + ln, L - 1), col = 16 * eb + ln, colc = min(col, E - 1);
+        const head_f32x4 acc = head_block_mma<true>(T + arow * TS, a.W, A, colc, A, kq);
+#pragma unroll
+        for (int i = 0; i < 4; ++i) {
+          const int row = 16 * rb + 4 * kq + i;
+          if (row < L && col < E) dYg[row * E + col] = acc[i];
+        }
+      } else {
+        const int u = t - n_dy, eb = u / nch, ch = u - eb * nch;
+        const int cb0 = ch * ncb / nch, ncw = (ch + 1) * ncb / nch - cb0;
+        const int e = min(16 * eb + ln, E - 1);
+        int colc[4];
+#pragma unroll
+        for (int c = 0; c < 4; ++c) colc[c] = min(16 * (cb0 + min(c, ncw - 1)) + ln, A - 1);
+        head_f32x4 acc[4];
+#pragma unroll
+        for (int c = 0; c < 4; ++c) acc[c] = head_f32x4{0.f, 0.f, 0.f, 0.f};
+        for (int st = 0; 4 * st < L; ++st) {
+          const int l = 4 * st + kq, lc = min(l, L - 1);
+          const float xa = Xs[lc * XS + e];
+          const float av = l < L ? xa : 0.f;
+          float bv[4];
+#pragma unroll
+          for (int c = 0; c < 4; ++c) bv[c] = T[lc * TS + colc[c]];
+#pragma unroll
+          for (int c = 0; c < 4; ++c)
+            if (c < ncw) acc[c] = __builtin_amdgcn_mfma_f32_16x16x4f32(av, bv[c], acc[c], 0, 0, 0);
+        }
+#pragma unroll
+        for (int c = 0; c < 4; ++c) {
+          const int col = 16 * (cb0 + c) + ln;
+#pragma unroll
+          for (int i = 0; i < 4; ++i) {
+            const int row = 16 * eb + 4 * kq + i;
+            if (c < ncw && row < E && col < A) dWg[row * A + col] = acc[c][i];
+          }
+        }
+      }
+    }
+  }
+}
+
+__global__ __launch_bounds__(HEAD_THREADS) void user_head_train_kernel(HeadArgs a) { user_head_body<false>(a); }
+__global__ __launch_bounds__(HEAD_THREADS) void user_head_dense_train_kernel(HeadArgs a) { user_head_body<true>(a); }
 
 __global__ __launch_bounds__(256) void user_head_finish_kernel(const float* __restrict__ partials, int64_t B, int A,
                                                                float* __restrict__ dq, float* __restrict__ db,
@@ -261,6 +437,10 @@
 size_t head_lds_bytes(int L, int C, int E, int A) {
   return sizeof(float) * (static_cast<size_t>(L) * A + static_cast<size_t>(L) * E + static_cast<size_t>(C) * E + 2 * static_cast<size_t>(E) +
                           2 * static_cast<size_t>(L) + 2 * static_cast<size_t>(C));
+}
+
+size_t head_dense_lds_bytes(int L, int C, int E, int A) {
+  return head_lds_bytes(L, C, E, A) + sizeof(float) * static_cast<size_t>(L) * ((head_row_stride(E) - E) + (head_row_stride(A) - A)) + 2 * sizeof(int);
 }
 
 }
@@ -291,7 +471,8 @@
   static const hipError_t attr = hipFuncSetAttribute(reinterpret_cast<const void*>(&user_head_train_kernel),
                                                      hipFuncAttributeMaxDynamicSharedMemorySize, 150 * 1024);
   if (attr != hipSuccess) return static_cast<int>(attr);
-  HeadArgs a{U, b, q, X, cand, labels, w, user, scores, probs, loss_rows, dcand, duser, de, partials, L, C, E, A, loss_kind, inv_batch};
+  HeadArgs a{U, b, q, X, cand, labels, w, user, scores, probs, loss_rows, dcand, duser, de, partials, L, C, E, A, loss_kind, inv_batch,
+             nullptr, nullptr, nullptr};
   EBN_LAUNCH(user_head_train_kernel, dim3(static_cast<unsigned>(B)), dim3(HEAD_THREADS), lds, s, a);
   EBN_CHECK_LAUNCH();
   if (dq == nullptr) return EBN_OK;
@@ -300,3 +481,49 @@
   EBN_CHECK_LAUNCH();
   return EBN_OK;
 }
+
+#define EBN_HEAD_DENSE_WS_CAP (int64_t{1} << 23)
+
+extern "C" int64_t ebn_user_head_dense_workspace_floats(int64_t B, int32_t E, int32_t A) {
+  if (!ebn_dim_ok(B, E, A)) return 0;
+  const int64_t n = ebn_sat_mul(ebn_sat_mul(B, E), A);
+  return n <= EBN_HEAD_DENSE_WS_CAP ? n : 0;
+}
+
+extern "C" int ebn_user_head_dense_supported(int64_t B, int32_t L, int32_t C, int32_t E, int32_t A, const float* W, const float* X,
+                                             const float* dY, const float* dW_parts) {
+  if (B < 0 || !ebn_user_head_supported(L, C, E, A)) return 0;
+  if (head_dense_lds_bytes(L, C, E, A) > 150 * 1024) return 0;
+  if (B > 0 && ebn_user_head_dense_workspace_floats(B, E, A) == 0) return 0;
+  return (ebn_aligned16(W) && ebn_aligned16(X) && ebn_aligned16(dY) && ebn_aligned16(dW_parts)) ? 1 : 0;
+}
+
+extern "C" int ebn_user_head_dense_train_f32(const float* W, const float* b, const float* q, const float* X, const float* cand,
+                                             const float* labels, float* w, float* user, float* scores, float* probs,
+                                             float* loss_rows, float* loss_out, float* dcand, float* duser, float* de, float* dq,
+                                             float* db, float* partials, float* dY, float* dW_parts, int64_t B, int32_t L, int32_t C,
+                                             int32_t E, int32_t A, int32_t loss_kind, float inv_batch, ebn_stream_t stream) {
+  EBN_REQUIRE(W && b && q && X && cand && labels && w && user && scores && probs && loss_rows && loss_out && dcand && duser && de &&
+                  partials && dY && dW_parts && ((dq != nullptr) == (db != nullptr)),
+              EBN_ERR_BAD_ARG);
+  EBN_REQUIRE(B >= 0 && L > 0 && C > 0 && E > 0 && A > 0, EBN_ERR_BAD_ARG);
+  EBN_REQUIRE(loss_kind >= 0 && loss_kind <= 2 && ebn_user_head_dense_supported(B, L, C, E, A, nullptr, nullptr, nullptr, nullptr),
+              EBN_ERR_UNSUPPORTED);
+  EBN_REQUIRE(ebn_aligned16(W) && ebn_aligned16(b) && ebn_aligned16(q) && ebn_aligned16(X) && ebn_aligned16(cand) && ebn_aligned16(user) &&
+                  ebn_aligned16(dcand) && ebn_aligned16(duser) && ebn_aligned16(dY) && ebn_aligned16(dW_parts),
+              EBN_ERR_ALIGN);
+  if (B == 0) return EBN_OK;
+  hipStream_t s = ebn_stream(stream);
+  static const hipError_t attr = hipFuncSetAttribute(reinterpret_cast<const void*>(&user_head_dense_train_kernel),
+                                                     hipFuncAttributeMaxDynamicSharedMemorySize, 150 * 1024);
+  if (attr != hipSuccess) return static_cast<int>(attr);
+  HeadArgs a{nullptr, b, q, X, cand, labels, w, user, scores, probs, loss_rows, dcand, duser, de, partials, L, C, E, A, loss_kind, inv_batch,
+             W, dY, dW_parts};
+  EBN_LAUNCH(user_head_dense_train_kernel, dim3(static_cast<unsigned>(B)), dim3(HEAD_THREADS), head_dense_lds_bytes(L, C, E, A), s, a);
+  EBN_CHECK_LAUNCH();
+  if (dq == nullptr) return EBN_OK;
+  EBN_LAUNCH(user_head_finish_kernel, dim3(static_cast<unsigned>(ebn_ceil_div(2 * A, 256) + 1)), dim3(256), 0, s, partials, B, A, dq, db,
+             loss_rows, loss_out);
+  EBN_CHECK_LAUNCH();
+  return EBN_OK;
+}
diff --git a/ebnerd-benchmark_amd/ebrec/models/newsrec/_engine.py b/ebnerd-benchmark_amd/ebrec/models/newsrec/_engine.py
--- a/ebnerd-benchmark_amd/ebrec/models/newsrec/_engine.py
+++ b/ebnerd-benchmark_amd/ebrec/models/newsrec/_engine.py
@@ -178,6 +178,8 @@
         self.loss_dev = torch.zeros(1, device=self.device)
         self.use_graph = False
         self.fuse_user_head = True
+        self.dense_user_head = False
+        self._dense_head_live = False
         self.fuse_eval_gather = True
         self.defer_finish = True
         self.atomic_table_grad = False
@@ -788,7 +790,19 @@
             ub.duser = torch.empty(ub.n_seq, E, device=self.device)
             ub.loss_rows = torch.empty(ub.n_seq, device=self.device)
             ub.head_partials = torch.empty(max(int(_hip.lib().ebn_user_head_partials_len(ub.n_seq, self.A)), 1), device=self.device)
+        if self.dense_user_head and getattr(ub, "dw_parts", None) is None:
+            n = int(_hip.lib().ebn_user_head_dense_workspace_floats(ub.n_seq, E, self.A))
+            ub.dw_parts = torch.empty(n, device=self.device) if n > 0 else False
         return nb, ub
+
+    def _dense_head(self, B, C, ub) -> bool:
+        parts = getattr(ub, "dw_parts", None)
+        if not (self.dense_user_head and self.fuse_user_head and self.mlp is None and self.precision == "exact"
+                and isinstance(parts, torch.Tensor) and self._fold_pooling(self.H)):
+            return False
+        pv = self.params.view
+        return int(_hip.lib().ebn_user_head_dense_supported(B, self.H, C, self.E, self.A, _hip.ptr(pv("u_W")), _hip.ptr(ub.Y), _hip.ptr(ub.dY),
+                                                            _hip.ptr(parts))) != 0
 
     SEG_KINDS = {"k": "kernels", "c": "collective", "a": "collective started asynchronously", "w": "wait for the started collectives"}
 
@@ -843,18 +857,19 @@
     def _adam_fused(self, C) -> bool:
         return bool(self.adam_in_finish and not self.multi and self._deferred(C))
 
-    def _adam_flat_args(self):
-        a = getattr(self, "_adam_flat", None)
+    def _adam_flat_args(self, dense_head=False):
+        cache = self.__dict__.setdefault("_adam_flat", {})
+        a = cache.get(bool(dense_head))
         if a is None:
             P = self.params
             a = _hip.AdamFlat()
             a.theta, a.grad, a.m, a.v, a.numel = P.data.data_ptr(), P.grad.data_ptr(), P.m.data_ptr(), P.v.data_ptr(), P.numel
             a.beta1, a.beta2, a.eps, a.grad_scale = BETA1, BETA2, ADAM_EPS, 1.0
-            rest = sorted((P.offsets[k], int(np.prod(P.shapes[k]))) for k in ("u_Wqkv", "u_W"))
+            rest = sorted((P.offsets[k], int(np.prod(P.shapes[k]))) for k in (("u_Wqkv",) if dense_head else ("u_Wqkv", "u_W")))
             a.n_rest = len(rest)
             for i, (off, n) in enumerate(rest):
                 a.rest_off[i], a.rest_len[i] = off, n
-            self._adam_flat = a
+            cache[bool(dense_head)] = a
         return a
 
     def _defer_bufs(self, nb):
@@ -874,16 +889,32 @@
         X, cand, dcand = nb.out, nb.out[B * H:], nb.dNE[B * H:]
         _hip.call("ebn_gemm_f32_site", 0, 0, R, 3 * E, E, one, _hip.ptr(X), E, _hip.ptr(pv("u_Wqkv")), 3 * E, zero, _hip.ptr(ub.QKV), 3 * E, ws, wsn, 1, S())
         _hip.call("ebn_attn_fwd_f32", _hip.ptr(ub.QKV), 3 * E, _hip.ptr(ub.Y), E, B, H, self.h, self.d, None, -1, zero, S())
+        self._dense_head_live = self._dense_head(B, C, ub)
+        if self._dense_head_live:
+            _hip.call("ebn_user_head_dense_train_f32", _hip.ptr(pv("u_W")), _hip.ptr(pv("u_b")), _hip.ptr(pv("u_q")), _hip.ptr(ub.Y), _hip.ptr(cand),
+                      _hip.ptr(nb.labels), _hip.ptr(ub.w), _hip.ptr(ub.out), _hip.ptr(nb.scores), _hip.ptr(nb.probs), _hip.ptr(ub.loss_rows),
+                      _hip.ptr(self.loss_dev), _hip.ptr(dcand), _hip.ptr(ub.duser), _hip.ptr(ub.de), None, None, _hip.ptr(ub.head_partials),
+                      _hip.ptr(ub.dY), _hip.ptr(ub.dw_parts), B, H, C, E, A, self.loss_kind, ctypes.c_float(1.0 / B), S())
+        else:
+            self._user_head_separate_matmuls(B, C, nb, ub)
+        _hip.call("ebn_attn_bwd_pooled_f32", _hip.ptr(ub.QKV), 3 * E, _hip.ptr(ub.dY), E, _hip.ptr(ub.w), _hip.ptr(ub.duser), E, _hip.ptr(ub.dQKV), 3 * E,
+                  B, H, self.h, self.d, None, -1, zero, S())
+        _hip.call("ebn_dense_bwd_pair_f32", R, E, 3 * E, _hip.ptr(X), E, _hip.ptr(ub.dQKV), 3 * E, _hip.ptr(pv("u_Wqkv")), 3 * E, zero, _hip.ptr(g("u_Wqkv")),
+                  3 * E, _hip.ptr(nb.dNE), E, ws, wsn, S())
+
+    def _user_head_separate_matmuls(self, B, C, nb, ub):
+        S, H, E, A = _hip.stream_handle, self.H, self.E, self.A
+        R = B * H
+        pv, g = self.params.view, self.params.g
+        ws, wsn = _hip.ptr(ub.ws), ub.ws.numel()
+        one, zero = ctypes.c_float(1.0), ctypes.c_float(0.0)
+        cand, dcand = nb.out[B * H:], nb.dNE[B * H:]
         _hip.call("ebn_gemm_f32_ws", 0, 0, R, A, E, one, _hip.ptr(ub.Y), E, _hip.ptr(pv("u_W")), A, zero, _hip.ptr(ub.U), A, ws, wsn, S())
         _hip.call("ebn_user_head_train_f32", _hip.ptr(ub.U), _hip.ptr(pv("u_b")), _hip.ptr(pv("u_q")), _hip.ptr(ub.Y), _hip.ptr(cand), _hip.ptr(nb.labels),
                   _hip.ptr(ub.w), _hip.ptr(ub.out), _hip.ptr(nb.scores), _hip.ptr(nb.probs), _hip.ptr(ub.loss_rows), _hip.ptr(self.loss_dev), _hip.ptr(dcand),
                   _hip.ptr(ub.duser), _hip.ptr(ub.de), None, None, _hip.ptr(ub.head_partials), B, H, C, E, A, self.loss_kind, ctypes.c_float(1.0 / B), S())
         _hip.call("ebn_dense_bwd_pair_f32", R, E, A, _hip.ptr(ub.Y), E, _hip.ptr(ub.U), A, _hip.ptr(pv("u_W")), A, zero, _hip.ptr(g("u_W")), A,
                   _hip.ptr(ub.dY), E, ws, wsn, S())
-        _hip.call("ebn_attn_bwd_pooled_f32", _hip.ptr(ub.QKV), 3 * E, _hip.ptr(ub.dY), E, _hip.ptr(ub.w), _hip.ptr(ub.duser), E, _hip.ptr(ub.dQKV), 3 * E,
-                  B, H, self.h, self.d, None, -1, zero, S())
-        _hip.call("ebn_dense_bwd_pair_f32", R, E, 3 * E, _hip.ptr(X), E, _hip.ptr(ub.dQKV), 3 * E, _hip.ptr(pv("u_Wqkv")), 3 * E, zero, _hip.ptr(g("u_Wqkv")),
-                  3 * E, _hip.ptr(nb.dNE), E, ws, wsn, S())
 
     def _news_bwd_deferred(self, nb, ub, B, N, part):
         S, E, A, T, D = _hip.stream_handle, self.E, self.A, self.T, self.D
@@ -910,17 +941,23 @@
             nb.finish_jobs["dWqkv"] = int(n.value)
             if part == "p2a":
                 return
-        jobs = (_hip.FinishJob * 4)()
+        dense = self._dense_head_live
+        n_jobs = 5 if dense else 4
+        jobs = (_hip.FinishJob * n_jobs)()
         jobs[0] = _hip.FinishJob(_hip.FINISH_COLRED, int(L.ebn_attpool_partials_len(R, A)) // (2 * A), 1, A, nb.partials.data_ptr(), g("n_q").data_ptr(),
                                  g("n_b").data_ptr(), A, 0.0, 1.0, None, None)
         jobs[1] = _hip.FinishJob(_hip.FINISH_HEAD, 1, B, A, ub.head_partials.data_ptr(), g("u_q").data_ptr(), g("u_b").data_ptr(), A, 0.0, 1.0,
                                  ub.loss_rows.data_ptr(), self.loss_dev.data_ptr())
-        jobs[2] = _hip.FinishJob(_hip.FINISH_SPLITK, nb.finish_jobs["dW"], E, A, nb.ws_dw.data_ptr(), g("n_W").data_ptr(), None, A, 0.0, 1.0, None, None)
-        jobs[3] = _hip.FinishJob(_hip.FINISH_SPLITK, nb.finish_jobs["dWqkv"], D, 3 * E, nb.ws_dwqkv.data_ptr(), g("n_Wqkv").data_ptr(), None, 3 * E, 0.0, 1.0, None, None)
+        nj = 2
+        if dense:
+            jobs[nj] = _hip.FinishJob(_hip.FINISH_SPLITK, B, E, A, ub.dw_parts.data_ptr(), g("u_W").data_ptr(), None, A, 0.0, 1.0, None, None)
+            nj += 1
+        jobs[nj] = _hip.FinishJob(_hip.FINISH_SPLITK, nb.finish_jobs["dW"], E, A, nb.ws_dw.data_ptr(), g("n_W").data_ptr(), None, A, 0.0, 1.0, None, None)
+        jobs[nj + 1] = _hip.FinishJob(_hip.FINISH_SPLITK, nb.finish_jobs["dWqkv"], D, 3 * E, nb.ws_dwqkv.data_ptr(), g("n_Wqkv").data_ptr(), None, 3 * E, 0.0, 1.0, None, None)
         if part == "p2b":
-            _hip.call("ebn_grad_finish_adam_f32", jobs, 4, ctypes.byref(self._adam_flat_args()), _hip.ptr(self.state), S())
+            _hip.call("ebn_grad_finish_adam_f32", jobs, n_jobs, ctypes.byref(self._adam_flat_args(dense)), _hip.ptr(self.state), S())
         else:
-            _hip.call("ebn_grad_finish_f32", jobs, 4, S())
+            _hip.call("ebn_grad_finish_f32", jobs, n_jobs, S())
 
     def _fwd_user_stage_kernels(self, B, C, nb, ub):
         H, E = self.H, self.E
@@ -934,11 +971,12 @@
         grads = _hip.EncoderGrads(g("u_Wqkv").data_ptr(), g("u_W").data_ptr(), g("u_b").data_ptr(), g("u_q").data_ptr())
         scratch = _hip.EncoderScratch(ub.dY.data_ptr(), ub.dQKV.data_ptr(), ub.de.data_ptr(), ub.partials.data_ptr(),
                                       ub.ws.data_ptr(), ub.ws.numel())
-        _hip.call("ebn_user_stage_train_f32", ctypes.byref(dims), ctypes.byref(params), ctypes.byref(acts), _hip.ptr(cand),
+        self._dense_head_live = self._dense_head(B, C, ub)
+        _hip.call("ebn_user_stage_dense_train_f32", ctypes.byref(dims), ctypes.byref(params), ctypes.byref(acts), _hip.ptr(cand),
                   _hip.ptr(nb.labels), _hip.ptr(nb.scores), _hip.ptr(nb.probs), _hip.ptr(ub.loss_rows), _hip.ptr(self.loss_dev),
                   _hip.ptr(dcand), _hip.ptr(ub.duser), ctypes.byref(grads), ctypes.byref(scratch),
-                  _hip.ptr(ub.head_partials) if self.fuse_user_head else None, _hip.ptr(nb.dNE), C, self.loss_kind,
-                  ctypes.c_float(1.0 / B), st, S())
+                  _hip.ptr(ub.head_partials) if self.fuse_user_head else None, _hip.ptr(ub.dw_parts) if self._dense_head_live else None,
+                  _hip.ptr(nb.dNE), C, self.loss_kind, ctypes.c_float(1.0 / B), st, S())
 
     def _accumulate_fixed(self, ids, dX, n_tok, st, site, p):
         _hip.call("ebn_embedding_grad_scatter_fixed_atomic" if self.atomic_table_grad else "ebn_embedding_grad_scatter_fixed", _hip.ptr(ids),
diff --git a/ebnerd-benchmark_amd/ebrec/models/newsrec/_engine_segments.py b/ebnerd-benchmark_amd/ebrec/models/newsrec/_engine_segments.py
--- a/ebnerd-benchmark_amd/ebrec/models/newsrec/_engine_segments.py
+++ b/ebnerd-benchmark_amd/ebrec/models/newsrec/_engine_segments.py
@@ -105,7 +105,7 @@
         return self.graph_collectives
 
     def _graph_key(self, B, C, advanced=False):
-        return (B, C, advanced, bool(self.adam_in_finish), bool(self.defer_finish), bool(self.multi))
+        return (B, C, advanced, bool(self.adam_in_finish), bool(self.defer_finish), bool(self.multi), bool(self.dense_user_head))
 
     def _capture(self, B, C, advanced=False):
         torch.cuda.synchronize()
diff --git a/include/ebnerd_hip.h b/include/ebnerd_hip.h
--- a/include/ebnerd_hip.h
+++ b/include/ebnerd_hip.h
@@ -112,6 +112,8 @@
   float* loss_out;
 } ebn_finish_job;
 int ebn_grad_finish_f32(const ebn_finish_job* jobs, int32_t n_jobs, ebn_stream_t stream);
+int ebn_splitk_sum_f32(const float* partials, int32_t n_parts, int64_t rows, int64_t cols, float beta, float* out, int64_t ld,
+                       ebn_stream_t stream);
 
 #define EBN_ADAM_FLAT_MAX_REST 12
 typedef struct ebn_adam_flat {
@@ -230,6 +232,11 @@
                              float* loss_out, float* dcand, float* duser, const ebn_encoder_grads* g,
                              const ebn_encoder_scratch* s, float* head_partials, float* dX, int32_t C, int32_t loss_kind,
                              float inv_batch, const ebn_step_state* st, ebn_stream_t stream);
+int ebn_user_stage_dense_train_f32(const ebn_encoder_dims* dims, const ebn_encoder_params* p, const ebn_encoder_acts* a,
+                                   const float* cand, const float* labels, float* scores, float* probs, float* loss_rows,
+                                   float* loss_out, float* dcand, float* duser, const ebn_encoder_grads* g,
+                                   const ebn_encoder_scratch* s, float* head_partials, float* dW_parts, float* dX, int32_t C,
+                                   int32_t loss_kind, float inv_batch, const ebn_step_state* st, ebn_stream_t stream);
 
 int ebn_score_fwd_f32(const float* cand, const float* user, float* scores, float* probs,
                       int64_t B, int32_t C, int32_t E, int32_t mode, ebn_stream_t stream);
@@ -247,6 +254,14 @@
                             float* dcand, float* duser, float* de, float* dq, float* db, float* partials, int64_t B,
                             int32_t L, int32_t C, int32_t E, int32_t A, int32_t loss_kind, float inv_batch,
                             ebn_stream_t stream);
+int64_t ebn_user_head_dense_workspace_floats(int64_t B, int32_t E, int32_t A);
+int ebn_user_head_dense_supported(int64_t B, int32_t L, int32_t C, int32_t E, int32_t A, const float* W, const float* X,
+                                  const float* dY, const float* dW_parts);
+int ebn_user_head_dense_train_f32(const float* W, const float* b, const float* q, const float* X, const float* cand,
+                                  const float* labels, float* w, float* user, float* scores, float* probs, float* loss_rows,
+                                  float* loss_out, float* dcand, float* duser, float* de, float* dq, float* db, float* partials,
+                                  float* dY, float* dW_parts, int64_t B, int32_t L, int32_t C, int32_t E, int32_t A,
+                                  int32_t loss_kind, float inv_batch, ebn_stream_t stream);
 int ebn_auc_hist_f32(const float* probs, const float* labels, int64_t n, const double* thresholds, int32_t n_thresholds,
                      int64_t* pos_hist, int64_t* neg_hist, ebn_stream_t stream);
 int ebn_pair_score_f32(const float* user, const float* news, const int32_t* u_idx,
```

Result: no change. 25710 (median of 3 runs) (-0.1%).
